# WhatAShot/Electrocardio-Panorama

Hardware: AMD Instinct MI355X
Metric: ECG-samples/sec (train step) (higher is better)
Workload: dtype f32 (conv products: fp32 operands split into fp16 hi+lo = 22-23 bits, block-scaled, 3 fp16 matrix products each, fp32 accumulate; fp32-class, not IEEE fp32)

## Files before the change

electrocardio_panorama_amd/_env.py:

```python
import os

PRODUCT = {
    "NEF_H2": "1 (default): K = 1 / 3 / 7 convolutions on the split-fp16 kernels; 0: the fp32 Winograd / direct kernels (strict fp32, "
              "required for data whose dynamic range exceeds ops.H2_HEADROOM per step)",
    "NEF_H2_TAIL": "warn (default): split-fp16 call sites whose operand is heavy-tailed (ops.H2_TAIL_FRAC) are counted and reported; "
                   "fp32: such WEIGHT-GRADIENT sites run on the fp32 kernels for their lifetime (per site, per rank)",
    "NEF_H2_ALLOW_CLAMP": "1: Solver warns instead of raising when a split-fp16 launch clamped outside a protected train step",
    "NEF_WINOGRAD": "fp32 path: 4 (default) F(4,.) forms where allowed, 2 / 1: F(2,.) only, 0: direct kernels only",
    "NEF_SIDE_STREAM": "auto (default) / 1 / 0: weight gradients on a second HIP stream",
    "NEF_SOLVER_GRAPH": "0: Solver never replays the captured step",
    "NEF_GRAPH_SPLIT": "0: data-parallel graphed step as ONE graph + one exposed all-reduce (default: two graphs, early bucket between them)",
    "NEF_EARLY_REDUCE": "0: eager data-parallel step reduces one bucket at the optimiser step (default: early bucket under the encoder's backward)",
    "NEF_BENCH_DUMP": "bench.py: file for the per-launch event times of the breakdown steps",
    "NEF_TIE_LOG": "tests: file for the tie ratios of the decision-replaying tests",
    "NEF_TEST_HOOKS": "1: honour the test hooks (TEST_HOOKS)",
}
TEST_HOOKS = {"NEF_SHARE_GPU", "NEF_DIST_BACKEND", "NEF_DIST_FORCE"}


def get(name, default=None):
    if name not in PRODUCT:
        raise KeyError(f"{name}: not a switch of this package (electrocardio_panorama_amd/_env.py)")
    return os.environ.get(name, default)
```

electrocardio_panorama_amd/_lib.py:

```python
import ctypes as C
import os

import torch

_HERE = os.path.dirname(os.path.abspath(__file__))
LIB_PATH = os.path.join(_HERE, "csrc", "libnefnet_hip.so")

NEF_OK = 0
_ERR = {-1: "NEF_E_SHAPE", -2: "NEF_E_NULL", -3: "NEF_E_WORKSPACE", -4: "NEF_E_UNSUPPORTED"}

p = C.c_void_p
i32 = C.c_int
i64 = C.c_int64
f32 = C.c_float
sz = C.c_size_t


class ConvArgs(C.Structure):
    _fields_ = [
        ("x", p), ("wp", p), ("y", p), ("bias", p), ("in_scale", p), ("res", p), ("gate", p), ("mask", p),
        ("x_bs", i64), ("x_gs", i64), ("y_bs", i64), ("y_gs", i64), ("sc_bs", i64), ("sc_gs", i64),
        ("res_bs", i64), ("res_gs", i64), ("gate_bs", i64), ("gate_gs", i64),
        ("B", i32), ("T", i32), ("G", i32), ("Cin_g", i32), ("Cout_g", i32), ("K", i32),
        ("relu", i32), ("gate_scale", f32), ("drop_scale", f32), ("drop_p", f32), ("rng_seed", C.c_uint64),
# ... 80 lines not shown


class LocateCandsArgs(C.Structure):
    _fields_ = [("best_theta", p), ("best_index", p), ("cands", p), ("s1", f32), ("s2", f32), ("ph1", f32), ("ph2", f32),
                ("B", i32), ("R", i32), ("radius", i32), ("reserved0", i32)]


class AugmentArgs(C.Structure):
    _fields_ = [("x", p), ("rois", p), ("y", p), ("seed_dev", p), ("seed", C.c_uint64),
                ("wander_amp", C.c_double), ("wander_lo", C.c_double), ("wander_hi", C.c_double), ("hum_amp", C.c_double),
                ("hum_hz", C.c_double), ("sample_rate", C.c_double), ("noise_std", f32), ("lead_drop", f32),
                ("B", i32), ("V", i32), ("L", i32), ("R", i32), ("crop", i32), ("reserved0", i32)]


class WarpArgs(C.Structure):
    _fields_ = [("data", p), ("target", p), ("rest", p), ("rois", p), ("data_out", p), ("target_out", p), ("rest_out", p),
                ("rois_out", p), ("seed", C.c_uint64), ("index0", i64), ("amp", C.c_double * 6),
                ("jitter", i32), ("B", i32), ("V", i32), ("R", i32), ("L", i32), ("reserved0", i32)]


class BeatBatchArgs(C.Structure):
    _fields_ = [("signal", p), ("plan", p), ("data", p), ("target_view", p), ("rest_view", p), ("signal_elems", i64),
                ("B", i32), ("V", i32), ("R", i32), ("dtype", i32)]


class BeatRangeArgs(C.Structure):
    _fields_ = [("signal", p), ("plan", p), ("range", p), ("signal_elems", i64), ("B", i32), ("V", i32), ("R", i32), ("dtype", i32)]


class BeatStitchArgs(C.Structure):
    _fields_ = [("views", p), ("range", p), ("table", p), ("out", p), ("view_bs", i64), ("view_as", i64), ("out_elems", i64),
                ("Bt", i32), ("A", i32), ("fill", i32), ("reserved0", i32)]


class RecordingStatsArgs(C.Structure):
    _fields_ = [("out", p), ("signal", p), ("beat_table", p), ("rec_table", p), ("out_offsets", p), ("score_leads", p), ("stats", p),
                ("out_elems", i64), ("signal_elems", i64), ("Bt", i32), ("N", i32), ("A", i32), ("fill", i32), ("dtype", i32),
                ("reserved0", i32)]


class PackDesc(C.Structure):
    _fields_ = [("w", p), ("wp", p), ("G", i32), ("Cog", i32), ("Cig", i32), ("K", i32), ("transpose_flip", i32),
                ("wino", i32), ("src_mode", i32), ("src_Cr", i32)]


SIGNATURES = {
    "nef_abi_version": (i32, []),
    "nef_debug_spin_us": (i32, [f32, i32, p]),
    "nef_stem_fwd": (i32, [p, p, p, i32, i32, i32, p]),
    "nef_stem_bwd_ws_bytes": (sz, [i32]),
    "nef_stem_bwd_weight": (i32, [p, p, p, p, p, sz, i32, i32, i32, p]),
    "nef_pack_weights": (i32, [C.POINTER(PackDesc), i32, p]),
    "nef_pack_bytes": (sz, [C.POINTER(PackDesc)]),
    "nef_conv_fwd": (i32, [C.POINTER(ConvArgs), p]),
    "nef_conv_args_bytes": (sz, []),
    "nef_conv_bwd_weight_ws_bytes": (sz, [C.POINTER(BwwArgs)]),
    "nef_conv_bwd_weight": (i32, [C.POINTER(BwwArgs), p]),
    "nef_bww_args_bytes": (sz, []),
    "nef_h2_tail_census_ws_bytes": (sz, [i32, i32, i32]),
    "nef_h2_tail_census": (i32, [p, i64, i64, i32, i32, i32, i32, p, i64, i64, p, p, i32, i32, p, f32, f32, p, sz, p, p, p, p]),
    "nef_bwd_weight_clamp_ends": (i32, [p, p, i64, i64, p, i32, i32, i32, i32, i32, p]),
    "nef_chan_sum_ws_bytes": (sz, [i32]),
    "nef_chan_sum": (i32, [p, p, p, sz, i32, i32, i32, p]),
    "nef_convt2_fwd": (i32, [p, p, p, p, i32, i32, i32, i32, i32, p]),
    "nef_convt2_bwd_data": (i32, [p, p, p, i32, i32, i32, i32, i32, p]),
    "nef_group_transpose": (i32, [p, p, i32, i32, i32, p]),
    "nef_convt2_interleave": (i32, [p, p, p, i32, i32, i32, p]),
    "nef_convt2_deinterleave": (i32, [p, p, i32, i32, i32, p]),
    "nef_convt2_bwd_weight_ws_bytes": (sz, [i32, i32, i32]),
    "nef_convt2_bwd_weight": (i32, [p, p, p, p, p, sz, i32, i32, i32, i32, i32, p]),
    "nef_theta_mlp_fwd": (i32, [p, p, p, p, i32, i32, p]),
    "nef_theta_mlp_bwd": (i32, [p, p, p, p, i32, i32, p]),
    "nef_theta_encode": (i32, [p, p, i32, p]),
    "nef_chscale_fwd": (i32, [p, p, i64, p, i32, i32, i32, p]),
    "nef_chscale_bwd": (i32, [p, p, p, i64, p, p, i32, i32, i32, i32, p]),
    "nef_gate": (i32, [p, p, p, f32, i64, p]),
    "nef_add": (i32, [p, p, p, i64, p]),
    "nef_roi_align_fwd": (i32, [p, p, p, i32, i32, i32, i32, i32, p]),
    "nef_roi_align_bwd": (i32, [p, p, p, i32, i32, i32, i32, i32, p]),
    "nef_window_crop": (i32, [p, i64, i64, p, i32, i32, i32, i32, i32, i32, p]),
    "nef_window_scatter": (i32, [p, p, i64, i64, i32, i32, i32, i32, i32, i32, p]),
    "nef_roi_unpool_fwd": (i32, [p, p, p, p, i32, i32, i32, p]),
    "nef_roi_unpool_bwd": (i32, [p, p, p, i32, i32, i32, p]),
    "nef_roi_segment_table": (i32, [p, p, p, i32, p]),
    "nef_lead_mean": (i32, [p, p, p, i32, i32, i32, p]),
    "nef_mix_fwd": (i32, [p, p, p, p, p, i32, i32, i32, i32, i32, p, p]),
    "nef_mix_bwd": (i32, [p, p, p, p, p, p, p, p, i32, i32, i32, i32, i32, p, i32, i32, i32, p]),
    "nef_mix_fwd_shared": (i32, [p, p, p, p, p, i32, i32, i32, i32, i32, p, p]),
    "nef_lead_mean_mix_shared": (i32, [p, p, p, p, p, i32, i32, i32, i32, i32, p, p]),
    "nef_lead_mean_mix_unpool": (i32, [p, p, p, p, p, p, p, i32, i32, i32, i32, i32, p, p]),
    "nef_mix_bwd_unpool": (i32, [p, p, p, p, p, p, p, p, p, i32, i32, i32, i32, i32, p, i32, p]),
    "nef_mix_bwd_unpool_rs": (i32, [p, p, p, p, p, p, p, p, p, p, p, sz, p, i32, i32, i32, i32, i32, p, i32, p]),
    "nef_mix_bwd_unpool_rs_ws_bytes": (sz, [i32, i32]),
    "nef_pass_combine_fwd": (i32, [p, p, p, i32, i32, i32, p]),
    "nef_pass_combine_bwd": (i32, [p, p, i32, i32, i32, p]),
    "nef_pass_combine_stats_ws_bytes": (sz, [i32, i32]),
    "nef_pass_combine_fwd_stats": (i32, [p, p, p, p, p, p, p, p, p, p, p, p, sz, i32, i32, i32, f32, f32, p, p]),
    "nef_upsample2_fwd": (i32, [p, p, i64, i32, p]),
    "nef_upsample2_bwd": (i32, [p, p, i64, i32, p]),
    "nef_bn_ws_bytes": (sz, [i32, i32]),
    "nef_bn_train_stats": (i32, [p, p, p, p, p, p, p, p, p, p, sz, i32, i32, i32, i32, f32, f32, p, p]),
    "nef_conv_stats_slots": (i32, [i32, i32]),
    "nef_bn_stats_from_slots": (i32, [p, i32, p, p, p, p, p, p, p, p, p, sz, i32, i32, i32, i32, f32, f32, p, p]),
    "nef_bn_eval_affine": (i32, [p, p, p, p, p, p, i32, f32, p]),
    "nef_fold_bn": (i32, [p, p, p, p, p, p, i32, i32, p]),
    "nef_affine_relu_fwd": (i32, [p, p, p, p, i32, i32, i32, i32, p]),
    "nef_bn_bwd_ws_bytes": (sz, [C.POINTER(BnBwdArgs)]),
    "nef_bn_relu_bwd": (i32, [C.POINTER(BnBwdArgs), p]),
    "nef_bn_bwd_args_bytes": (sz, []),
    "nef_bn_relu_bwd_outconv_w": (i32, [C.POINTER(BnBwdArgs), p, p, p, sz, p]),
# ... 141 lines not shown
```

electrocardio_panorama_amd/csrc/conv_h2.hip:

```cpp
#include <hip/hip_runtime.h>
#include <stdint.h>
#include <stdlib.h>

#include "nefnet_hip.h"
#include "nef_common.h"


typedef float f32x16 __attribute__((ext_vector_type(16)));
typedef float f32x4 __attribute__((ext_vector_type(4)));
typedef float f32x2 __attribute__((ext_vector_type(2)));
typedef float f32x4_a4 __attribute__((ext_vector_type(4), aligned(4)));
typedef _Float16 h16x8 __attribute__((ext_vector_type(8)));
typedef _Float16 h16x2 __attribute__((ext_vector_type(2)));
typedef unsigned u32x4 __attribute__((ext_vector_type(4)));
typedef unsigned u32x2 __attribute__((ext_vector_type(2)));

namespace {

constexpr int KC = 16;
constexpr int NTO = 256;
constexpr int PRO_MAX_CIN = 512;

__device__ __forceinline__ void split2(float x0, float x1, unsigned& h, unsigned& l) {
    x0 = __builtin_amdgcn_fmed3f(x0, -65000.f, 65000.f);
// ... 38 lines not shown
    const float* const wr = d.w + (r * d.Cig + ci) * 3;
    const float w0 = wr[0], w1 = wr[1], w2 = wr[2];
    if (p == 0) return kk == 0 ? fmaf(0.75f, w0, 0.25f * w1) : (kk == 1 ? fmaf(0.25f, w0, 0.75f * (w1 + w2)) : 0.25f * w2);
    return kk == 0 ? 0.25f * w0 : (kk == 1 ? fmaf(0.25f, w2, 0.75f * (w0 + w1)) : fmaf(0.75f, w2, 0.25f * w1));
}
constexpr int H2_PACK_MAX = 48;
struct H2PackTable { H2PackDesc d[H2_PACK_MAX]; };

__global__ __launch_bounds__(256) void pack_h2_kernel(H2PackTable tab) {
    const H2PackDesc& d = tab.d[blockIdx.y];
    const int co_n = d.flip ? d.Cig : d.Cog;
    const int ci_n = d.flip ? d.Cog : d.Cig;
    const int K = d.K;
    const int lane = threadIdx.x & 63;
    const int rows = d.G * co_n;
    const int ncot = co_n / 32, nc16 = ci_n / 16;
    float* const dsc = reinterpret_cast<float*>(d.wp + (int64_t)d.G * K * co_n * ci_n * 2);
    for (int row = blockIdx.x * 4 + (threadIdx.x >> 6); row < rows; row += gridDim.x * 4) {
        const int g = row / co_n, co = row % co_n;
        float m = 0.f;
        for (int i = lane; i < ci_n * K; i += 64) {
            const int ci = i / K, kk = i % K;
            const float v = d.flip ? h2_pack_src(d, (int64_t)g * d.Cog + ci, co, K - 1 - kk) : h2_pack_src(d, (int64_t)g * d.Cog + co, ci, kk);
            m = fmaxf(m, fabsf(v));
        }
#pragma unroll
        for (int o = 32; o > 0; o >>= 1) m = fmaxf(m, __shfl_xor(m, o, 64));
        int e = 0;
        if (m > 0.f && m < 3e38f) {
            int ex;
            (void)frexpf(m, &ex);
            e = 14 - (ex - 1);
            e = e > 100 ? 100 : (e < -100 ? -100 : e);
        }
        const float sc = ldexpf(1.f, e);
        if (lane == 0) dsc[row] = ldexpf(1.f, -e);
        for (int i = lane; i < ci_n * K; i += 64) {
            const int ci = i / K, kk = i % K;
            const float v = sc * (d.flip ? h2_pack_src(d, (int64_t)g * d.Cog + ci, co, K - 1 - kk) : h2_pack_src(d, (int64_t)g * d.Cog + co, ci, kk));
            const _Float16 h = (_Float16)v;
            const _Float16 l = (_Float16)(v - (float)h);
            const int64_t frag = ((((int64_t)g * nc16 + ci / 16) * K + kk) * ncot + co / 32) * 2;
            const int fl = (co & 31) + 32 * ((ci & 15) >> 3);
            d.wp[(frag * 64 + fl) * 8 + (ci & 7)] = h;
            d.wp[((frag + 1) * 64 + fl) * 8 + (ci & 7)] = l;
        }
    }
}

#define NEF_H2_TRACK1(V) amax_ = fmaxf(amax_, fabsf(V));
#define NEF_H2_TRACK2(V, W) amax_ = fmaxf(amax_, fmaxf(fabsf(V), fabsf(W)));
constexpr int H2_OCC1 = 3;
template <int K, int PRO, int TM, bool PACK = false>
__global__ __launch_bounds__(256, (TM == 1 && (PRO & 2) == 0) ? H2_OCC1 : 2) void conv_h2_kernel(nef_conv_args a_, int tps_, int n_tiles_, int m_tiles_) {
    constexpr int MT = 64 * TM;
    constexpr bool UP = (PRO & 2) != 0, AFF = (PRO & 1) != 0;
    constexpr bool PH = (PRO & 4) != 0;
    static_assert(!PH || (!UP && K == 3), "phase-stacked input: K = 3, no upsampling prologue");
    constexpr bool PF = (PRO & 8) != 0;
    static_assert(!PF || (!UP && !PH && K == 3 && TM == 2 && !PACK), "polyphase forward: K = 3, 128-row tile");
    constexpr int NS = UP ? 2 : 1;
    constexpr int PAD = (K - 1) / 2;
    constexpr int XROW = NTO + K - 1;
    constexpr int P4 = (XROW + 3) / 4 + 1;
    constexpr int PLANE = 4 * P4 * 32;
    constexpr int HALF = 4 * P4 * 16;
#define NEF_H2_WADDR(R, W) (((W) >> 1) * HALF + (((R) & 3) * P4 + ((R) >> 2)) * 16 + ((W) & 1) * 8)
#define NEF_H2_RPOS(S) ((((S) & 3) * P4 + ((S) >> 2)) * 16)
    constexpr int NIT = (XROW + 63) / 64;
    constexpr int NSF = K + 3;
    extern __shared__ __attribute__((aligned(16))) unsigned char smem_h2[];
    unsigned char* const Xl = smem_h2;
    float* const Pl = reinterpret_cast<float*>(smem_h2 + 4 * PLANE);
    float* const El = Pl + (AFF ? 2 * PRO_MAX_CIN : 0);
    float* const Al = El + 8 * MT;

    typedef const nef_conv_args __attribute__((address_space(4))) kargs_t;
    auto tile_pass = [&](kargs_t* const ap, const int bid, const int tid, const int tps, const int n_tiles, const int m_tiles,
                         const float xs_force, const bool last) __attribute__((always_inline)) -> float {
#define a (*ap)
    const int tile = bid % n_tiles;
    const int gm = bid / n_tiles;
    const int mt = gm % m_tiles;
    const int g = gm / m_tiles;
    int b0, t0;
    if constexpr (PACK) {
        b0 = tile * tps;
        t0 = 0;
    } else {
        const int full = (n_tiles / (8 * tps)) * (8 * tps);
        if (tile < full) {
            const int grp = tile / (8 * tps), r = tile % (8 * tps);
            b0 = grp * 8 + (r & 7);
            t0 = (r >> 3) * NTO;
        } else {
            b0 = tile / tps;
            t0 = (tile - b0 * tps) * NTO;
        }
    }
    const int m0 = mt * MT;
    const int T = a.T, Cig = a.Cin_g, Cog = a.Cout_g;
    const int lane = tid & 63, wave = tid >> 6;
    const int lo = lane & 31, hi = lane >> 5;
    const int wave_u = __builtin_amdgcn_readfirstlane(wave);
    const int wm = wave_u >> 1, wn = wave_u & 1;
    const int Tin = UP ? (T >> 1) : (PH ? 2 * T : T);

    const float* const xbase = a.x + (int64_t)b0 * a.x_bs + (int64_t)g * a.x_gs;
    const __amdgpu_buffer_rsrc_t xrs = nef_rsrc(xbase);
    const _Float16* const wph = reinterpret_cast<const _Float16*>(a.wp);
    const int ncot = Cog / 32, nc16 = Cig / 16;
    const __amdgpu_buffer_rsrc_t wrs = nef_rsrc(wph + ((int64_t)g * nc16 * K * ncot * 2 + (int64_t)(m0 / 32 + TM * wm) * 2) * 512);
    const unsigned a_tap = (unsigned)(ncot * 2 * 1024);

    const int64_t soff = (int64_t)b0 * a.sc_bs + (int64_t)g * a.sc_gs;
    float xs_ = xs_force;
    if (!last) {
        xs_ = a.x_scale != 0.f ? a.x_scale : 1.f;
        if (a.x_amax) {
            const float m_ = a.x_amax[0];
            if (m_ > 0.f && m_ < 3e38f) {
                int e_;
                (void)frexpf(m_, &e_);
                xs_ = ldexpf(1.f, 9 - e_ < 100 ? 9 - e_ : 100);
            }
        }
    }
    const int pro_row0 = AFF ? (b0 / a.pro_Bp) * a.G * Cig + g * Cig : 0;
    const unsigned avo = (unsigned)(lane * 16);
    unsigned xvo[NIT][NS];
    float lam[NIT];
    bool xok[NIT];
#pragma unroll
    for (int it = 0; it < NIT; ++it) {
        const int r = lane + 64 * it;
        const int t = t0 + r - PAD;
        xok[it] = (r < XROW) && (t >= 0) && (t < T);
        lam[it] = 0.f;
        if constexpr (PACK) {
            const int v = r - PAD, vb = v >= 0 ? v / (T + 4) : 0, tl = v - vb * (T + 4);
            xok[it] = (r < XROW) && v >= 0 && tl < T && vb < tps && b0 + vb < a.B;
            xvo[it][0] = xok[it] ? (unsigned)((vb * (int)a.x_bs + tl) * 4) : NEF_OOB;
        } else if constexpr (UP) {
            float src = 0.5f * ((float)t + 0.5f) - 0.5f;
            if (src < 0.f) src = 0.f;
            int i0 = (int)src;
            if (i0 > Tin - 1) i0 = Tin - 1;
            const int i1 = i0 + (i0 < Tin - 1 ? 1 : 0);
            lam[it] = src - (float)i0;
            xvo[it][0] = xok[it] ? (unsigned)(i0 * 4) : NEF_OOB;
            xvo[it][NS - 1] = xok[it] ? (unsigned)(i1 * 4) : NEF_OOB;
        } else if constexpr (PF) {
            xok[it] = (r < XROW) && (t >= -1) && (t <= T);
            const int tc = t < 0 ? 0 : (t > T - 1 ? T - 1 : t);
            xvo[it][0] = xok[it] ? (unsigned)(tc * 4) : NEF_OOB;
        } else {
            xvo[it][0] = xok[it] ? (unsigned)(t * (PH ? 8 : 4)) : NEF_OOB;
        }
    }
    unsigned uvo[2][2], mvo[2];
    bool uok[2][2], mok[2];
    float ulam[2];
    if constexpr (UP) {
        static_assert(!UP || (K == 3 && NTO == 256), "interval staging: K = 3, 256-column tiles");
#pragma unroll
// ... 116 lines not shown
                v *= sa_[rr];                                                                                       \
                NEF_H2_TRACK1(v)                                                                                    \
                v_[rr] = v;                                                                                         \
            }                                                                                                       \
            const int r = lane + 64 * it;                                                                           \
            unsigned h0_, l0_, h1_, l1_;                                                                            \
            split2n(v_[0], v_[1], h0_, l0_);                                                                        \
            split2n(v_[2], v_[3], h1_, l1_);                                                                        \
            const u32x2 hv = {h0_, h1_}, lv = {l0_, l1_};                                                           \
            if (r < XROW) {                                                                                         \
                unsigned char* p_ = (BUFP) + NEF_H2_WADDR(r, wave);                                                 \
                *reinterpret_cast<u32x2*>(p_) = hv;                                                                 \
                *reinterpret_cast<u32x2*>(p_ + PLANE) = lv;                                                         \
            }                                                                                                       \
        }                                                                                                           \
    }
    h16x8 fa[2][2 * TM];
#define NEF_H2A_ISSUE(CH, KK, SET)                                                                                   \
    {                                                                                                               \
        const unsigned so_ = (unsigned)(((CH) * K + (KK)) * a_tap);                                                 \
        _Pragma("unroll") for (int q = 0; q < 2 * TM; ++q)                                                          \
            fa[SET][q] = __builtin_bit_cast(h16x8, nef_buf_f32x4(wrs, avo, so_ + (unsigned)(q * 1024)));            \
    }

    NEF_H2X_ISSUE(0, xrs)
    NEF_H2A_ISSUE(0, 0, 0)
    if (tid < MT) {
        const int ch_ = g * Cog + m0 + (int)tid;
        const float* const dsc = reinterpret_cast<const float*>(wph + (int64_t)a.G * K * Cog * Cig * 2);
        if constexpr (PF) El[tid] = a.bias ? a.bias[g * (Cog >> 1) + (m0 >> 1) + ((int)tid >> 6) * 32 + ((int)tid & 31)] : 0.f;
        else
        El[tid] = a.bias ? a.bias[ch_] : 0.f;
        El[5 * MT + tid] = dsc[ch_] / xs_;
        El[6 * MT + tid] = (a.res_scale && b0 < a.B) ? a.res_scale[(int64_t)b0 * a.rs_bs + (int64_t)g * a.rs_gs + m0 + (int)tid] : 1.f;
        El[7 * MT + tid] = (a.gate_rowscale && b0 < a.B) ? a.gate_rowscale[(int64_t)b0 * a.gr_bs + (int64_t)g * a.gr_gs + m0 + (int)tid] : 1.f;
        if (a.bnb_slots) {
            const int pr_ = (b0 / a.bnb_Bp) * a.G * Cog + ch_;
            El[MT + tid] = a.bnb_mean[pr_];
            El[2 * MT + tid] = a.bnb_invstd[pr_];
            El[3 * MT + tid] = a.bnb_a[pr_];
            El[4 * MT + tid] = a.bnb_b[pr_];
        }
    }
    if constexpr (AFF) {
        for (int i = tid; i < Cig; i += 256) {
            Pl[i] = a.pro_a[pro_row0 + i];
            Pl[Cig + i] = a.pro_b[pro_row0 + i];
        }
        __syncthreads();
    }
    NEF_H2X_STORE(0, Xl)
    __syncthreads();

    const int nst = Cig / KC;
    const unsigned fb_lane = (unsigned)(hi * HALF + (wn * 32 + lo) * 16);
    for (int st = 0; st < nst; ++st) {
        const unsigned char* const xb = Xl + (st & 1) * (2 * PLANE) + fb_lane;
        const bool more = st + 1 < nst;
        const __amdgpu_buffer_rsrc_t xrs_n = nef_rsrc_n(xbase, more ? 0x7FFFFFFCu : 0u);
        h16x8 fb[5][2];
#define NEF_H2B_LOAD(S)                                                                                              \
    {                                                                                                               \
        const unsigned char* p_ = xb + NEF_H2_RPOS(S);                                                              \
        fb[(S) % 5][0] = *reinterpret_cast<const h16x8*>(p_);                                                       \
        fb[(S) % 5][1] = *reinterpret_cast<const h16x8*>(p_ + PLANE);                                               \
    }
        NEF_H2B_LOAD(0)
        NEF_H2B_LOAD(1)
        NEF_H2B_LOAD(2)
        NEF_H2B_LOAD(3)
#pragma unroll
        for (int kk = 0; kk < K; ++kk) {
            if (kk + 1 < K) NEF_H2A_ISSUE(st, kk + 1, (kk + 1) & 1)
            else NEF_H2A_ISSUE(more ? st + 1 : st, 0, (kk + 1) & 1)
            if (kk == 0) {
                __builtin_amdgcn_sched_barrier(0);
                NEF_H2X_ISSUE((st + 1) * KC, xrs_n)
            }
            if (kk + 4 < NSF) NEF_H2B_LOAD(kk + 4)
            __builtin_amdgcn_s_setprio(1);
            const int s_ = kk & 1;
#pragma unroll
            for (int j = 0; j < 4; ++j)
#pragma unroll
                for (int i = 0; i < TM; ++i)
                    acc[i][j] = __builtin_amdgcn_mfma_f32_32x32x16_f16(fa[s_][2 * i], fb[(kk + j) % 5][0], acc[i][j], 0, 0, 0);
#pragma unroll
            for (int j = 0; j < 4; ++j)
#pragma unroll
                for (int i = 0; i < TM; ++i)
                    acc[i][j] = __builtin_amdgcn_mfma_f32_32x32x16_f16(fa[s_][2 * i], fb[(kk + j) % 5][1], acc[i][j], 0, 0, 0);
#pragma unroll
            for (int j = 0; j < 4; ++j)
#pragma unroll
                for (int i = 0; i < TM; ++i)
                    acc[i][j] = __builtin_amdgcn_mfma_f32_32x32x16_f16(fa[s_][2 * i + 1], fb[(kk + j) % 5][0], acc[i][j], 0, 0, 0);
        }
#undef NEF_H2B_LOAD
        if constexpr ((K & 1) != 0) {
#pragma unroll
            for (int q = 0; q < 2 * TM; ++q) fa[0][q] = fa[1][q];
        }
        if (more) NEF_H2X_STORE((st + 1) * KC, Xl + ((st + 1) & 1) * (2 * PLANE))
        else {
#pragma unroll
            for (int o = 32; o > 0; o >>= 1) amax_ = fmaxf(amax_, __shfl_xor(amax_, o, 64));
            amax_ *= 1.f / xs_;
            if (lane == 0) Al[wave_u] = amax_;
        }
        __syncthreads();
    }
    {
        const float wg_ = fmaxf(fmaxf(Al[0], Al[1]), fmaxf(Al[2], Al[3]));
        if (!last && !(wg_ * xs_ < 65000.f) && wg_ < 3e38f) {
            __syncthreads();
            return wg_;
        }
    }
#undef NEF_H2X_ISSUE
#undef NEF_H2X_STORE
#undef NEF_H2A_ISSUE
#undef NEF_H2_WADDR
#undef NEF_H2_RPOS

    if (a.x_clamped && lane == 0 && !(amax_ * xs_ < 65000.f)) atomicAdd(a.x_clamped, 1);
    if (a.x_amax_next) {
        if (lane == 0 && amax_ < 3e38f) {
            unsigned* const p_ = reinterpret_cast<unsigned*>(a.x_amax_next);
            const unsigned b_ = __builtin_bit_cast(unsigned, amax_);
            if (b_ > __atomic_load_n(p_, __ATOMIC_RELAXED)) atomicMax(p_, b_);
        }
    }
    if constexpr (PF) {
        const int t = t0 + wn * 128 + 4 * lo;
        const bool inb = b0 < a.B;
        const bool live0 = inb && t < T, live1 = inb && t + 2 < T;
        const int Cr = Cog >> 1;
        const int cw = (m0 >> 1) + wm * 32;
        const int erow = wm * 64 + 4 * hi;
        const __amdgpu_buffer_rsrc_t yrs = nef_rsrc(a.y + (int64_t)b0 * a.y_bs + (int64_t)g * a.y_gs + (int64_t)cw * (2 * T));
        const unsigned yv0 = live0 ? (unsigned)((4 * hi * 2 * T + 2 * t) * 4) : NEF_OOB;
        const unsigned yv1 = live1 ? (unsigned)((4 * hi * 2 * T + 2 * t + 4) * 4) : NEF_OOB;
        float* const slot_out = a.stats;
        float sv[32];
#pragma unroll
        for (int h = 0; h < 2; ++h) {
#pragma unroll
            for (int q = 0; q < 8; ++q) {
                const int row = ((q + 8 * h) & 3) + 8 * ((q + 8 * h) >> 2);
                const float ds0 = El[5 * MT + erow + row], ds1 = El[5 * MT + erow + 32 + row], bv = El[erow + row];
                float y0[4], y1[4];
#pragma unroll
                for (int e = 0; e < 4; ++e) {
                    y0[e] = fmaf(acc[0][e][q + 8 * h], ds0, bv);
                    y1[e] = fmaf(acc[TM - 1][e][q + 8 * h], ds1, bv);
                }
                const f32x4 o0 = {y0[0], y1[0], y0[1], y1[1]}, o1 = {y0[2], y1[2], y0[3], y1[3]};
                nef_buf_store_f32x4(o0, yrs, yv0, (unsigned)(row * 2 * T * 4));
                nef_buf_store_f32x4(o1, yrs, yv1, (unsigned)(row * 2 * T * 4));
                if (slot_out) {
                    const float s0 = live0 ? (y0[0] + y1[0]) + (y0[1] + y1[1]) : 0.f, s1 = live1 ? (y0[2] + y1[2]) + (y0[3] + y1[3]) : 0.f;
                    const float q0 = live0 ? fmaf(y0[0], y0[0], y1[0] * y1[0]) + fmaf(y0[1], y0[1], y1[1] * y1[1]) : 0.f;
                    const float q1 = live1 ? fmaf(y0[2], y0[2], y1[2] * y1[2]) + fmaf(y0[3], y0[3], y1[3] * y1[3]) : 0.f;
                    sv[2 * (q + 8 * h)] = s0 + s1;
                    sv[2 * (q + 8 * h) + 1] = q0 + q1;
                }
// ... 192 lines not shown
            } else if (a.bnb_slots) {
                const float* xp = a.bnb_x + ((int64_t)b0 * ctot + (int64_t)g * Cog + cobase) * T;
#pragma unroll
                for (int q = 0; q < 8; ++q) {
                    const int row = NEF_ROW(q);
                    const int er = erow0 + row;
                    const float af = El[3 * MT + er], bf = El[4 * MT + er];
                    const float mf = El[MT + er], is = El[2 * MT + er];
                    const f32x2 x01 = *reinterpret_cast<const f32x2*>(xp + (int64_t)row * T + ts[0]);
                    const f32x2 x23 = *reinterpret_cast<const f32x2*>(xp + (int64_t)row * T + ts[1]);
                    const float g0 = (live[0] && fmaf(x01[0], af, bf) > 0.f) ? y[q][0] : 0.f;
                    const float g1 = (live[0] && fmaf(x01[1], af, bf) > 0.f) ? y[q][1] : 0.f;
                    const float g2 = (live[1] && fmaf(x23[0], af, bf) > 0.f) ? y[q][2] : 0.f;
                    const float g3 = (live[1] && fmaf(x23[1], af, bf) > 0.f) ? y[q][3] : 0.f;
                    sv[2 * (q + 8 * h)] = (g0 + g1) + (g2 + g3);
                    sv[2 * (q + 8 * h) + 1] = fmaf(g0, (x01[0] - mf) * is, g1 * ((x01[1] - mf) * is)) +
                                              fmaf(g2, (x23[0] - mf) * is, g3 * ((x23[1] - mf) * is));
                }
            } else if (a.stats && a.stats_mode == 0) {
#pragma unroll
                for (int q = 0; q < 8; ++q) {
                    const float y0 = live[0] ? y[q][0] : 0.f, y1 = live[0] ? y[q][1] : 0.f;
                    const float y2 = live[1] ? y[q][2] : 0.f, y3 = live[1] ? y[q][3] : 0.f;
                    sv[2 * (q + 8 * h)] = (y0 + y1) + (y2 + y3);
                    sv[2 * (q + 8 * h) + 1] = fmaf(y0, y0, y1 * y1) + fmaf(y2, y2, y3 * y3);
                }
            }
#undef NEF_ROW
        }
        if (slot_out) {
#pragma unroll
            for (int step = 0; step < 5; ++step) {
                const int off = 16 >> step;
                const bool up = (lo & off) != 0;
#pragma unroll
                for (int k = 0; k < off; ++k) {
                    const float send = up ? sv[k] : sv[k + off];
                    const float keep = up ? sv[k + off] : sv[k];
                    sv[k] = keep + __shfl_xor(send, off, 64);
                }
            }
            const int r = lo >> 1;
            const int ch = g * Cog + cobase + (r & 3) + 8 * (r >> 2);
            const int64_t nslot = (int64_t)tps * 2;
            const int64_t slot = (int64_t)b0 * nslot + (int64_t)(t0 / NTO) * 2 + wn;
            if (inb) slot_out[((int64_t)ch * a.B * nslot + slot) * 2 + (lo & 1)] = sv[0];
        }
    }
    return -1.f;
#undef a
    };
    kargs_t* ap_ = (kargs_t*)__builtin_amdgcn_kernarg_segment_ptr();
    (void)a_;
    const float over_ = tile_pass(ap_, (int)blockIdx.x, (int)threadIdx.x, tps_, n_tiles_, m_tiles_, 0.f, false);
    if (over_ > 0.f) {
        int e_;
        (void)frexpf(over_, &e_);
        int bid_ = (int)blockIdx.x, tid_ = (int)threadIdx.x, tps2_ = tps_, nt2_ = n_tiles_, mt2_ = m_tiles_;
        asm volatile("" : "+s"(ap_), "+s"(bid_), "+s"(tps2_), "+s"(nt2_), "+s"(mt2_));
        asm volatile("" : "+v"(tid_));
        (void)tile_pass(ap_, bid_, tid_, tps2_, nt2_, mt2_, ldexpf(1.f, 9 - e_ < 100 ? 9 - e_ : 100), true);
    }
}

template <int K, int PRO, int TM, bool PACK = false>
int launch_h2(const nef_conv_args& a, hipStream_t st) {
    constexpr int MT = 64 * TM;
    constexpr int XROW = NTO + K - 1;
    constexpr int P4 = (XROW + 3) / 4 + 1;
    constexpr int PLANE = 4 * P4 * 32;
    constexpr size_t lds = (size_t)4 * PLANE + (((PRO & 1) ? 2 * PRO_MAX_CIN : 0) + 8 * MT + 4) * sizeof(float);
    static unsigned long long lds_set = 0;
    if (int e = nef_ensure_dyn_lds(reinterpret_cast<const void*>(&conv_h2_kernel<K, PRO, TM, PACK>), lds, &lds_set)) return e;
    const int tps = PACK ? (NTO + 4) / (a.T + 4) : (a.T + NTO - 1) / NTO;
    const int n_tiles = PACK ? (a.B + tps - 1) / tps : a.B * tps;
    const int m_tiles = a.Cout_g / MT;
    const int64_t blocks = (int64_t)a.G * m_tiles * n_tiles;
    if (blocks <= 0 || blocks > 0x7fffffff) return NEF_E_SHAPE;
    hipLaunchKernelGGL((conv_h2_kernel<K, PRO, TM, PACK>), dim3((unsigned)blocks), dim3(256), lds, st, a, tps, n_tiles, m_tiles);
    return nef_launch_status();
}

}

static bool h2_pack_shape(const nef_conv_args* a) {
    if (!(a->T >= 8 && a->T <= 64 && a->T % 4 == 0 && (a->K == 1 || a->K == 3))) return false;
    const int64_t spt = (NTO + 4) / (a->T + 4);
    const int64_t lim = 0x7fffffff / 4;
    return a->pro_mode == 0 && !a->in_scale && !a->res_scale && !a->gate_rowscale && !a->stats && !a->bnb_slots && spt * a->x_bs < lim && spt * a->y_bs < lim &&
           (!a->res || spt * a->res_bs < lim) && (!a->gate || spt * a->gate_bs < lim);
}

__attribute__((visibility("hidden"))) bool nef_h2_ok(const nef_conv_args* a) {
    return (a->K == 1 || a->K == 3 || a->K == 7) && a->Cout_g % 64 == 0 && a->Cin_g % KC == 0 && a->T % 2 == 0 &&
           (a->T >= NTO / 2 || h2_pack_shape(a)) &&
           ((a->pro_mode >= 0 && a->pro_mode <= 4) || a->pro_mode == 8 || a->pro_mode == 9) && (a->K == 3 || a->pro_mode == 0) &&
           !(a->pro_mode && a->in_scale) &&
           (!a->res_scale || (a->res && !(a->pro_mode & 8))) &&
           ((!a->gate_rowscale && a->stats_mode == 0) || (a->gate && !(a->pro_mode & 8) && (a->stats_mode == 0 || (a->stats_mode == 1 && a->stats && !a->bnb_slots)))) &&
           (!(a->pro_mode & 8) || (a->Cout_g % 128 == 0 && a->T >= NTO / 2 && !a->res && !a->gate && !a->mask && !a->relu && a->drop_p <= 0.f &&
                                   !a->bnb_slots && (int64_t)a->Cout_g * a->T * 4 < 0x7fffffff)) &&
           (a->pro_mode != 4 || (a->T >= NTO / 2 && (int64_t)a->Cin_g * a->T * 4 < 0x7fffffff)) &&
           (!(a->pro_mode & 1) || a->Cin_g <= PRO_MAX_CIN);
}

__attribute__((visibility("hidden"))) int nef_h2_launch(const nef_conv_args* a, hipStream_t st) {
    if (!nef_h2_ok(a)) return NEF_E_SHAPE;
    if ((a->pro_mode & 1) && !(a->pro_a && a->pro_b && a->pro_Bp > 0)) return NEF_E_NULL;
    const bool wide = a->Cout_g % 128 == 0;
    if (a->T < NTO / 2)
        return a->K == 1 ? launch_h2<1, 0, 1, true>(*a, st) : launch_h2<3, 0, 1, true>(*a, st);
    if (a->K == 7) return wide ? launch_h2<7, 0, 2>(*a, st) : launch_h2<7, 0, 1>(*a, st);
    if (a->K == 1) return wide ? launch_h2<1, 0, 2>(*a, st) : launch_h2<1, 0, 1>(*a, st);
    switch (a->pro_mode) {
        case 0: return wide ? launch_h2<3, 0, 2>(*a, st) : launch_h2<3, 0, 1>(*a, st);
        case 1: return wide ? launch_h2<3, 1, 2>(*a, st) : launch_h2<3, 1, 1>(*a, st);
        case 2: return launch_h2<3, 2, 1>(*a, st);
        case 4: return wide ? launch_h2<3, 4, 2>(*a, st) : launch_h2<3, 4, 1>(*a, st);
        case 8: return launch_h2<3, 8, 2>(*a, st);
        case 9: return launch_h2<3, 9, 2>(*a, st);
        default: return launch_h2<3, 3, 1>(*a, st);
    }
}

__attribute__((visibility("hidden"))) int nef_h2_pack_status(const nef_pack_desc* dp) {
    const nef_pack_desc& d = *dp;
    const int co_n = d.transpose_flip ? d.Cig : d.Cog, ci_n = d.transpose_flip ? d.Cog : d.Cig;
    if (d.G <= 0 || co_n % 32 != 0 || ci_n % 16 != 0 || (d.K != 1 && d.K != 3 && d.K != 7)) return NEF_E_SHAPE;
    if (d.src_mode != 0 && !(d.src_mode == 1 && d.K == 3 && d.Cog % 2 == 0 && d.src_Cr >= 0 &&
                             (d.src_Cr == 0 || (d.src_Cr % 64 == 0 && d.Cog == 2 * d.src_Cr)))) return NEF_E_SHAPE;
    return NEF_OK;
}

__attribute__((visibility("hidden"))) int nef_h2_pack(const nef_pack_desc* descs, int n, hipStream_t st) {
    for (int i0 = 0; i0 < n; i0 += H2_PACK_MAX) {
        H2PackTable tab;
        const int m = n - i0 < H2_PACK_MAX ? n - i0 : H2_PACK_MAX;
        int rows_max = 1;
        for (int i = 0; i < m; ++i) {
            const nef_pack_desc& d = descs[i0 + i];
            if (!d.w || !d.wp) return NEF_E_NULL;
            if (int e = nef_h2_pack_status(&d)) return e;
            const int co_n = d.transpose_flip ? d.Cig : d.Cog;
            tab.d[i] = H2PackDesc{d.w, reinterpret_cast<_Float16*>(d.wp), d.G, d.Cog, d.Cig, d.K, d.transpose_flip, d.src_mode, d.src_Cr};
            if (d.G * co_n > rows_max) rows_max = d.G * co_n;
        }
        hipLaunchKernelGGL(pack_h2_kernel, dim3((unsigned)((rows_max + 3) / 4), (unsigned)m), dim3(256), 0, st, tab);
    }
    return nef_launch_status();
}
```

electrocardio_panorama_amd/csrc/conv_h2w.hip:

```cpp
#include <hip/hip_runtime.h>
#include <stdint.h>
#include <stdlib.h>

#include <type_traits>

#include "nefnet_hip.h"
#include "nef_common.h"


typedef float f32x16 __attribute__((ext_vector_type(16)));
typedef float f32x2 __attribute__((ext_vector_type(2)));
typedef _Float16 h16x8 __attribute__((ext_vector_type(8)));
typedef _Float16 h16x2 __attribute__((ext_vector_type(2)));
typedef unsigned u32x4 __attribute__((ext_vector_type(4)));
typedef unsigned u32x2 __attribute__((ext_vector_type(2)));

namespace {

constexpr int TT = 64;
constexpr int GP = TT * 2 + 8;
constexpr int XW = TT + 8;
constexpr int XP = XW * 2 + 8;
constexpr int X_PLANE = 64 * XP;
constexpr int gy_plane(int MCO) { return 64 * MCO * GP; }
constexpr int buf_bytes(int MCO) { return 2 * gy_plane(MCO) + 2 * X_PLANE; }

struct H2WArgs {
    const float* x;
    const float* gy;
    const float* in_scale;
    const float* pro_a;
    const float* pro_b;
    float* ws;
    const float* x_amax;
    const float* gy_amax;
    float* x_amax_next;
    float* gy_amax_next;
    int* clamped;
    int64_t x_bs, x_gs, gy_bs, gy_gs, sc_bs, sc_gs;
    int64_t x_end, gy_end;
    int B, T, G, Cig, Cog, pro_Bp, S, tps, n_tiles, m_tiles, c_tiles, teams;
    float x_scale, gy_scale;
    int xclamp;
};


__device__ __forceinline__ void split_pair_s(float x0, float x1, float s, unsigned& h, unsigned& l) {
    asm("v_fma_mixlo_f16 %0, %1, %2, 0 op_sel:[0,0,0] op_sel_hi:[0,0,0]" : "=v"(h) : "v"(x0), "v"(s));
    asm("v_fma_mixhi_f16 %0, %1, %2, 0 op_sel:[0,0,0] op_sel_hi:[0,0,0]" : "+v"(h) : "v"(x1), "v"(s));
    asm("v_fma_mixlo_f16 %0, %1, %2, -%3 op_sel:[0,0,0] op_sel_hi:[0,0,1]" : "=v"(l) : "v"(x0), "v"(s), "v"(h));
    asm("v_fma_mixhi_f16 %0, %1, %2, -%3 op_sel:[0,0,1] op_sel_hi:[0,0,1]" : "+v"(l) : "v"(x1), "v"(s), "v"(h));
}
__device__ __forceinline__ void split_one_s(float x0, float s, unsigned& h, unsigned& l) {
    asm("v_fma_mixlo_f16 %0, %1, %2, 0 op_sel:[0,0,0] op_sel_hi:[0,0,0]" : "=v"(h) : "v"(x0), "v"(s));
    asm("v_fma_mixlo_f16 %0, %1, %2, -%3 op_sel:[0,0,0] op_sel_hi:[0,0,1]" : "=v"(l) : "v"(x0), "v"(s), "v"(h));
}

__device__ __forceinline__ float scale_for(float m) {
    int e;
    (void)frexpf(m, &e);
    return ldexpf(1.f, 9 - e);
}

__device__ __forceinline__ float scale_from(const float* amax, float fallback) {
    float s = fallback != 0.f ? fallback : 1.f;
    if (amax) {
        const float m = amax[0];
        if (m > 0.f && m < 3e38f) {
            int e;
            (void)frexpf(m, &e);
            s = ldexpf(1.f, 9 - e);
        }
    }
    return s;
}

template <int K, int K0, int K1, int MCO, int KA>
__device__ __forceinline__ void h2w_chunk(const unsigned char* ga, const unsigned char* xa, int c, f32x16 (&acc)[MCO][KA]) {
    constexpr int PAD = (K - 1) / 2;
    constexpr int GY_PLANE = gy_plane(MCO);
    h16x8 fah[MCO], fal[MCO];
#pragma unroll
    for (int i = 0; i < MCO; ++i) {
        unsigned ah[4], al[4];
#pragma unroll
        for (int j = 0; j < 2; ++j) {
            const u32x2 vh = *reinterpret_cast<const u32x2*>(ga + i * 32 * GP + c * 32 + 8 * j);
            const u32x2 vl = *reinterpret_cast<const u32x2*>(ga + i * 32 * GP + GY_PLANE + c * 32 + 8 * j);
            ah[2 * j] = vh[0], ah[2 * j + 1] = vh[1];
            al[2 * j] = vl[0], al[2 * j + 1] = vl[1];
        }
        fah[i] = __builtin_bit_cast(h16x8, u32x4{ah[0], ah[1], ah[2], ah[3]});
        fal[i] = __builtin_bit_cast(h16x8, u32x4{al[0], al[1], al[2], al[3]});
    }
    unsigned wh[8], wl[8];
#pragma unroll
    for (int j = 0; j < 4; ++j) {
// ... 303 lines not shown
        if (e0 & 1) {
            fbh[k] = __builtin_bit_cast(h16x8, u32x4{wo_h[d], wo_h[d + 1], wo_h[d + 2], wo_h[d + 3]});
            fbl[k] = __builtin_bit_cast(h16x8, u32x4{wo_l[d], wo_l[d + 1], wo_l[d + 2], wo_l[d + 3]});
        } else {
            fbh[k] = __builtin_bit_cast(h16x8, u32x4{wn_h[d], wn_h[d + 1], wn_h[d + 2], wn_h[d + 3]});
            fbl[k] = __builtin_bit_cast(h16x8, u32x4{wn_l[d], wn_l[d + 1], wn_l[d + 2], wn_l[d + 3]});
        }
    }
#pragma unroll
    for (int i = 0; i < WR; ++i)
#pragma unroll
        for (int k = 0; k < K; ++k) acc[i][k] = __builtin_amdgcn_mfma_f32_32x32x16_f16(fah[i], fbh[k], acc[i][k], 0, 0, 0);
#pragma unroll
    for (int i = 0; i < WR; ++i)
#pragma unroll
        for (int k = 0; k < K; ++k) acc[i][k] = __builtin_amdgcn_mfma_f32_32x32x16_f16(fal[i], fbh[k], acc[i][k], 0, 0, 0);
#pragma unroll
    for (int i = 0; i < WR; ++i)
#pragma unroll
        for (int k = 0; k < K; ++k) acc[i][k] = __builtin_amdgcn_mfma_f32_32x32x16_f16(fah[i], fbl[k], acc[i][k], 0, 0, 0);
}

template <int K, int PRO, int WM, int WN, int WR, int TTv, int NP, int DEPTH>
__global__ __launch_bounds__(64 * (WM / WR * WN + NP), 1) void conv_h2w2_kernel(H2WArgs a) {
    constexpr bool UP = (PRO & 2) != 0, AFF = (PRO & 1) != 0;
    constexpr int NC = WM / WR * WN;
    constexpr int NT = 64 * NP, RG = 32 * WM, RX = 32 * WN;
    constexpr int GP = TTv * 2 + 16, XE = TTv + 8, XP = XE * 2;
    constexpr int G_PLANE = RG * GP, X_PLANE = RX * XP, BUF = 2 * G_PLANE + 4 * X_PLANE;
    constexpr int QG = TTv / 4, QX = XE / 4, NGQ = RG * QG / NT, NXQ = (RX * QX + NT - 1) / NT, NCH = TTv / 16;
    constexpr int GROWS = NT / QG;
    static_assert(RG * QG % NT == 0 && GP % 32 == 16 && XP % 32 == 16, "tile form");
    extern __shared__ __attribute__((aligned(16))) unsigned char smem_w[];

    const int members = a.m_tiles * a.c_tiles;
    const int xcd = blockIdx.x & 7, q_ = blockIdx.x >> 3;
    const int member = q_ % members;
    const int team = (q_ / members) * 8 + xcd;
    if (team >= a.teams) return;
    const int g = team / a.S, sp = team % a.S;
    const int mt = member / a.c_tiles, ct = member % a.c_tiles;
    const int T = a.T, Tin = UP ? (T >> 1) : T;
    const int lane = (int)threadIdx.x & 63;
    const int lo = lane & 31, hi = lane >> 5;
    const int wave_u = __builtin_amdgcn_readfirstlane((int)threadIdx.x >> 6);
    const int wm = (wave_u % NC) / WN * WR, wn = wave_u % WN;
    const bool producer = wave_u >= NC;
    const int tid = ((int)threadIdx.x - 64 * NC) & (NT - 1);

    const int64_t per = ((int64_t)a.n_tiles + a.S - 1) / a.S;
    const int n_lo = (int)(per * sp);
    int n_hi = (int)(per * (sp + 1));
    if (n_hi > a.n_tiles) n_hi = a.n_tiles;

    float* const Wl = reinterpret_cast<float*>(smem_w);
    float rx_ = 0.f, rg_ = 0.f;
    auto share_pass = [&](const float sx, const float sg, const bool last) __attribute__((always_inline)) -> bool {
    float amax_x = 0.f, amax_g = 0.f;

    f32x16 acc[WR][K];
#pragma unroll
    for (int i = 0; i < WR; ++i)
#pragma unroll
        for (int k = 0; k < K; ++k)
#pragma unroll
            for (int r = 0; r < 16; ++r) acc[i][k][r] = 0.f;

    const int g_row = tid / QG, g_qd = tid % QG;
    const unsigned g_voff = (unsigned)((g_row * T + 4 * g_qd) * 4);
    const unsigned g_lds = (unsigned)(g_row * GP + g_qd * 8);
    unsigned x_voff[NXQ], x_lds[NXQ], x_row[NXQ], x_qd[NXQ];
#pragma unroll
    for (int q = 0; q < NXQ; ++q) {
        const int p = tid + NT * q;
        const int row = p < RX * QX ? p / QX : 0, qd = p < RX * QX ? p % QX : 0;
        x_row[q] = (unsigned)row, x_qd[q] = (unsigned)qd;
        x_voff[q] = p < RX * QX ? (unsigned)((row * Tin + (UP ? 2 : 4) * qd) * 4) : NEF_OOB;
        x_lds[q] = (unsigned)(row * XP + qd * 8);
    }
    const bool has_sc = a.in_scale != nullptr;

    struct Stage {
        f32x4 gq[NGQ];
        f32x4 xq[NXQ];
        float x5[NXQ], ppa[NXQ], ppb[NXQ], psc[NXQ];
    };
    Stage st0, st1;

    auto is_edge = [&](int N) { const int t0_ = (N % a.tps) * TTv; return !(t0_ > 0 && t0_ + TTv + 6 <= T); };

    auto issue = [&](Stage& z, int N, auto edge_c, int part) __attribute__((always_inline)) {
        constexpr bool EDGE = decltype(edge_c)::value;
        const int b_ = N / a.tps, t0_ = (N % a.tps) * TTv;
        const bool on_ = N < n_hi;
        const int64_t goff = (int64_t)b_ * a.gy_bs + (int64_t)g * a.gy_gs + (int64_t)(mt * RG) * T + (EDGE ? 0 : t0_);
        const __amdgpu_buffer_rsrc_t grs = nef_rsrc_n(a.gy + goff, extent_from(a.gy_end, goff, on_));
#pragma unroll
        for (int q = 0; q < ((part & 1) ? NGQ : 0); ++q) {
            const unsigned so = (unsigned)(q * GROWS * T * 4);
            if constexpr (!EDGE) {
                z.gq[q] = nef_buf_f32x4(grs, g_voff, so);
            } else {
#pragma unroll
                for (int i = 0; i < 4; ++i) {
                    const int t = t0_ + 4 * g_qd + i;
                    z.gq[q][i] = nef_buf_f32(grs, t < T ? g_voff + (unsigned)((t0_ + i) * 4) : NEF_OOB, so);
                }
            }
        }
        const int64_t xrow0 = (int64_t)b_ * a.x_bs + (int64_t)g * a.x_gs + (int64_t)(ct * RX) * Tin;
        const int64_t xoff = xrow0 + (EDGE ? 0 : (UP ? (t0_ - 4) / 2 - 1 : t0_ - 4));
        const __amdgpu_buffer_rsrc_t xrs = nef_rsrc_n(a.x + xoff, extent_from(a.x_end, xoff, on_));
#pragma unroll
        for (int q = 0; q < ((part & 2) ? NXQ : 0); ++q) {
            if constexpr (!EDGE) {
                z.xq[q] = nef_buf_f32x4(xrs, x_voff[q], 0);
                if constexpr (!UP) z.x5[q] = nef_buf_f32(xrs, x_voff[q], 16);
            } else {
                const unsigned rowoff = x_voff[q] - (unsigned)((UP ? 2 : 4) * 4) * x_qd[q];
                const bool live = x_voff[q] != NEF_OOB;
                const int t = t0_ - 4 + 4 * (int)x_qd[q];
                if constexpr (UP) {
                    const int h_ = t >> 1;
#pragma unroll
                    for (int i = 0; i < 4; ++i) {
                        int c_ = h_ - 1 + i;
                        c_ = c_ < 0 ? 0 : (c_ > Tin - 1 ? Tin - 1 : c_);
                        z.xq[q][i] = nef_buf_f32(xrs, live && t + 4 >= 0 && t < T ? rowoff + (unsigned)(c_ * 4) : NEF_OOB, 0);
                    }
                } else {
#pragma unroll
                    for (int i = 0; i < 5; ++i) {
                        int ti = t + i;
                        if (a.xclamp) ti = ti == -1 ? 0 : (ti == T ? T - 1 : ti);
                        const float v = nef_buf_f32(xrs, live && ti >= 0 && ti < T ? rowoff + (unsigned)(ti * 4) : NEF_OOB, 0);
                        if (i < 4) z.xq[q][i] = v; else z.x5[q] = v;
                    }
                }
            }
            const int bq = on_ ? b_ : 0;
            if constexpr (AFF) {
                const int pr = (bq / a.pro_Bp) * a.G * a.Cig + g * a.Cig + ct * RX;
                z.ppa[q] = a.pro_a[pr + (int)x_row[q]], z.ppb[q] = a.pro_b[pr + (int)x_row[q]];
            }
            if (has_sc) z.psc[q] = a.in_scale[(int64_t)bq * a.sc_bs + (int64_t)g * a.sc_gs + ct * RX + (int)x_row[q]];
        }
    };

    auto store = [&](Stage& z, int N, unsigned char* bufp, auto edge_c, int part) __attribute__((always_inline)) {
        constexpr bool EDGE = decltype(edge_c)::value;
        const int t0_ = (N % a.tps) * TTv;
#pragma unroll
        for (int q = 0; q < ((part & 1) ? NGQ : 0); ++q) {
            const f32x4 v = z.gq[q];
            amax_g = fmaxf(amax_g, fmaxf(fabsf(v[0]), fabsf(v[1])));
            amax_g = fmaxf(amax_g, fmaxf(fabsf(v[2]), fabsf(v[3])));
            unsigned h0, l0, h1, l1;
            split_pair_s(v[0], v[1], sg, h0, l0);
            split_pair_s(v[2], v[3], sg, h1, l1);
            unsigned char* p_ = bufp + g_lds + q * GROWS * GP;
            *reinterpret_cast<u32x2*>(p_) = u32x2{h0, h1};
            *reinterpret_cast<u32x2*>(p_ + G_PLANE) = u32x2{l0, l1};
        }
#pragma unroll
        for (int q = 0; q < ((part & 2) ? NXQ : 0); ++q) {
            if (tid + NT * q < RX * QX) {
                float v[5];
                if constexpr (UP) {
                    float s0 = z.xq[q][0], s1 = z.xq[q][1], s2 = z.xq[q][2], s3 = z.xq[q][3];
                    if constexpr (AFF) {
                        s0 = fmaxf(fmaf(s0, z.ppa[q], z.ppb[q]), 0.f), s1 = fmaxf(fmaf(s1, z.ppa[q], z.ppb[q]), 0.f);
                        s2 = fmaxf(fmaf(s2, z.ppa[q], z.ppb[q]), 0.f), s3 = fmaxf(fmaf(s3, z.ppa[q], z.ppb[q]), 0.f);
                    }
                    v[0] = (1.f - 0.75f) * s0 + 0.75f * s1;
                    v[1] = (1.f - 0.25f) * s1 + 0.25f * s2;
                    v[2] = (1.f - 0.75f) * s1 + 0.75f * s2;
                    v[3] = (1.f - 0.25f) * s2 + 0.25f * s3;
                    v[4] = (1.f - 0.75f) * s2 + 0.75f * s3;
                    if constexpr (EDGE) {
                        if (t0_ - 4 + 4 * (int)x_qd[q] == 0) v[0] = s1;
                        if (t0_ + 4 * (int)x_qd[q] == 0) v[4] = s3;
                    }
                } else {
                    v[0] = z.xq[q][0], v[1] = z.xq[q][1], v[2] = z.xq[q][2], v[3] = z.xq[q][3], v[4] = z.x5[q];
                    if constexpr (AFF) {
#pragma unroll
                        for (int i = 0; i < 5; ++i) v[i] = fmaxf(fmaf(v[i], z.ppa[q], z.ppb[q]), 0.f);
                    }
                }
                if (has_sc) {
#pragma unroll
                    for (int i = 0; i < 5; ++i) v[i] *= z.psc[q];
                }
                if constexpr (EDGE) {
                    const int t = t0_ - 4 + 4 * (int)x_qd[q];
                    const int lo_ = a.xclamp ? -1 : 0, hi_ = a.xclamp ? T + 1 : T;
#pragma unroll
                    for (int i = 0; i < 5; ++i)
                        if (t + i < lo_ || t + i >= hi_) v[i] = 0.f;
                }
                amax_x = fmaxf(amax_x, fmaxf(fabsf(v[0]), fabsf(v[1])));
                amax_x = fmaxf(amax_x, fmaxf(fabsf(v[2]), fabsf(v[3])));
                unsigned h0, l0, h1, l1, h2, l2;
                split_pair_s(v[0], v[1], sx, h0, l0);
// ... 100 lines not shown
        for (int k = 0; k < K; ++k)
#pragma unroll
            for (int r = 0; r < 16; ++r) wsp[((int64_t)k * a.Cog + co0 + (r & 3) + 8 * (r >> 2)) * a.Cig + ci] = acc[i][k][r] * ds;
    }
    return true;
    };
    const float sx0 = scale_from(a.x_amax, a.x_scale), sg0 = scale_from(a.gy_amax, a.gy_scale);
    if (!share_pass(sx0, sg0, false))
        (void)share_pass(rx_ * sx0 < 65000.f ? sx0 : scale_for(rx_), rg_ * sg0 < 65000.f ? sg0 : scale_for(rg_), true);
}

template <int K, int PRO, int WM, int WN, int WR, int TTv, int NP, int DEPTH>
int launch_h2w2(const H2WArgs& a, hipStream_t st) {
    constexpr size_t lds = 2 * (2 * (32 * WM) * (TTv * 2 + 16) + 4 * (32 * WN) * ((TTv + 8) * 2));
    static unsigned long long lds_set = 0;
    if (int e = nef_ensure_dyn_lds(reinterpret_cast<const void*>(&conv_h2w2_kernel<K, PRO, WM, WN, WR, TTv, NP, DEPTH>), lds, &lds_set)) return e;
    const int members = a.m_tiles * a.c_tiles;
    const int teams8 = (a.teams + 7) / 8 * 8;
    const int64_t blocks = (int64_t)teams8 * members;
    if (blocks <= 0 || blocks > 0x7fffffff) return NEF_E_SHAPE;
    hipLaunchKernelGGL((conv_h2w2_kernel<K, PRO, WM, WN, WR, TTv, NP, DEPTH>), dim3((unsigned)blocks), dim3(64 * (WM / WR * WN + NP)), lds, st, a);
    return nef_launch_status();
}

int h2w2_form(int Cog, int pro_mode) {
    if (Cog % 128 == 0) return 1;
    return ((H2W2_64_MODES >> pro_mode) & 1) ? 2 : 0;
}

}

extern "C" {

__attribute__((visibility("hidden"))) bool nef_h2w_ok(int B, int T, int Cig, int Cog, int K, int pro_mode) {
    return (K == 1 || K == 3 || K == 7) && B > 0 && T >= TT && T % 2 == 0 && Cig % 64 == 0 && Cog % 64 == 0 && pro_mode >= 0 &&
           (pro_mode <= 3 || (pro_mode <= 5 && Cog % 128 == 0)) && (K == 3 || pro_mode == 0);
}

__attribute__((visibility("hidden"))) int nef_h2w_splits(int B, int T, int G, int Cig, int Cog, int K, int pro_mode, int* partials) {
    const int v2 = h2w2_form(Cog, pro_mode & 3);
    const H2WForm f = h2w_form(Cog, K);
    const int tps = (T + TT - 1) / TT;
    const int64_t n_tiles = (int64_t)B * tps;
    const int units = v2 ? G * (Cog / (v2 == 1 ? 128 : 64)) * (Cig / 64) : G * (Cog / (64 * f.mco)) * (Cig / 64);
    const int resident = v2 ? 1 : (f.split ? 1 : 2);
    const int slots = resident * nef_cu_count();
    int S = slots / units;
    if (S > n_tiles) S = (int)n_tiles;
    if (S < 1) S = 1;
    if (partials) *partials = S * (!v2 && f.split == 2 ? 2 : 1);
    return S;
}

__attribute__((visibility("hidden"))) int nef_h2w_launch(const nef_bww_args& b, int S, hipStream_t st) {
    const int B = b.B, T = b.T, G = b.G, Cig = b.Cin_g, Cog = b.Cout_g, K = b.K;
    int pro_mode = b.pro_mode;
    if (!nef_h2w_ok(B, T, Cig, Cog, K, pro_mode)) return NEF_E_SHAPE;
    if ((b.x_amax_next == nullptr) != (b.gy_amax_next == nullptr)) return NEF_E_NULL;
    const H2WForm f = h2w_form(Cog, K);
    H2WArgs a;
    a.x = b.x, a.gy = b.gy, a.in_scale = b.in_scale, a.pro_a = b.pro_a, a.pro_b = b.pro_b, a.ws = (float*)b.ws;
    a.x_amax = b.x_amax, a.gy_amax = b.gy_amax, a.x_amax_next = b.x_amax_next, a.gy_amax_next = b.gy_amax_next, a.clamped = b.clamped;
    a.x_bs = b.x_bs, a.x_gs = b.x_gs, a.gy_bs = b.gy_bs, a.gy_gs = b.gy_gs, a.sc_bs = b.sc_bs, a.sc_gs = b.sc_gs;
    a.B = B, a.T = T, a.G = G, a.Cig = Cig, a.Cog = Cog, a.pro_Bp = b.pro_Bp, a.S = S;
    a.tps = (T + TT - 1) / TT;
    a.n_tiles = B * a.tps;
    a.m_tiles = Cog / (64 * f.mco), a.c_tiles = Cig / 64;
    a.teams = G * S;
    a.x_scale = b.x_scale, a.gy_scale = b.gy_scale;
    a.xclamp = (pro_mode >> 2) & 1;
    pro_mode &= 3;
    const int Tin = (pro_mode & 2) ? T / 2 : T;
    a.x_end = ((int64_t)(B - 1) * b.x_bs + (int64_t)(G - 1) * b.x_gs + (int64_t)Cig * Tin) * 4;
    a.gy_end = ((int64_t)(B - 1) * b.gy_bs + (int64_t)(G - 1) * b.gy_gs + (int64_t)Cog * T) * 4;
    if (a.xclamp && !h2w2_form(Cog, pro_mode)) return NEF_E_UNSUPPORTED;
    if (const int v2 = h2w2_form(Cog, pro_mode)) {
        a.m_tiles = Cog / (v2 == 1 ? 128 : 64), a.c_tiles = Cig / 64;
#define NEF_H2W2(KK, PP)                                                                                             \
    (v2 == 1 ? launch_h2w2<KK, PP, 4, 2, (KK == 7 ? 1 : 2), 64, (KK == 7 ? 4 : 8), (KK == 7 ? 1 : 2)>(a, st)               \
             : launch_h2w2<KK, PP, 2, 2, 1, 64, 8, (KK == 7 ? 1 : 2)>(a, st))
        if (K == 7) return NEF_H2W2(7, 0);
        if (K == 1) return NEF_H2W2(1, 0);
        switch (pro_mode) {
            case 0: return NEF_H2W2(3, 0);
            case 1: return NEF_H2W2(3, 1);
            case 2: return NEF_H2W2(3, 2);
            default: return NEF_H2W2(3, 3);
        }
#undef NEF_H2W2
    }
    if (K == 7) return launch_h2w<7, 0, 1, 0>(a, st);
    if (K == 1) return launch_h2w<1, 0, 1, 0>(a, st);
    return pro_mode == 0 ? launch_h2w<3, 0, 1, 0>(a, st) : launch_h2w<3, 1, 1, 0>(a, st);
}

}
```

electrocardio_panorama_amd/csrc/conv_mfma.hip:

```cpp
#include "nef_common.h"
#include <stdlib.h>

typedef float f32x16 __attribute__((ext_vector_type(16)));
typedef float f32x4 __attribute__((ext_vector_type(4)));
typedef float f32x2 __attribute__((ext_vector_type(2)));

#ifndef NEF_MFMA_PART
#define NEF_MFMA_PART 0
#endif
#define NEF_PART(n) (NEF_MFMA_PART == 0 || NEF_MFMA_PART == (n))

namespace {

constexpr int NT = 128;
constexpr int WT = 64;

template <int K> struct StageK;
template <> struct StageK<7> { static constexpr int KC = 16; };
template <int K, int TM> struct FwdStage {
    static constexpr int KC = ((K == 7 || K == 3) && TM == 2) ? 8 : StageK<K>::KC;
};
template <> struct StageK<3> { static constexpr int KC = 16; };
template <> struct StageK<1> { static constexpr int KC = 64; };

// ... 1882 lines not shown
        else pack_plain_elem(d.w, d.wp, d.G, d.Cog, d.Cig, d.K, d.transpose_flip, i);
    }
}

__global__ void chan_sum_partial(const float* __restrict__ x, double* __restrict__ part, int B, int C, int T,
                                 int nsplit) {
    __shared__ double sm[4];
    const int c = blockIdx.x % C;
    const int sp = blockIdx.x / C;
    double s = 0.0;
    const int nb = sp < B ? (B - sp + nsplit - 1) / nsplit : 0;
    if (T >= 512 && (T & 1) == 0) {
        const int T2 = T >> 1;
        int bi = 0;
        for (; bi + 4 <= nb; bi += 4) {
            const float2* r0 = reinterpret_cast<const float2*>(x + ((int64_t)(sp + bi * nsplit) * C + c) * T);
            const int64_t rs = (int64_t)nsplit * C * T2;
            for (int t = threadIdx.x; t < T2; t += blockDim.x) {
                const float2 a0 = r0[t], a1 = r0[rs + t], a2 = r0[2 * rs + t], a3 = r0[3 * rs + t];
                s += ((double)a0.x + (double)a0.y) + ((double)a1.x + (double)a1.y) +
                     (((double)a2.x + (double)a2.y) + ((double)a3.x + (double)a3.y));
            }
        }
        for (; bi < nb; ++bi) {
            const float2* r0 = reinterpret_cast<const float2*>(x + ((int64_t)(sp + bi * nsplit) * C + c) * T);
            for (int t = threadIdx.x; t < T2; t += blockDim.x) {
                const float2 a0 = r0[t];
                s += (double)a0.x + (double)a0.y;
            }
        }
    } else {
        for (int i = threadIdx.x; i < nb * T; i += blockDim.x) {
            const int bi = i / T, t = i - bi * T;
            s += (double)x[((int64_t)(sp + bi * nsplit) * C + c) * T + t];
        }
    }
    s = nef_block_sum_d(s, sm);
    if (threadIdx.x == 0) part[(int64_t)sp * C + c] = s;
}

__global__ void chan_sum_final(const double* __restrict__ part, float* __restrict__ out, int C, int nsplit) {
    const int c = blockIdx.x * blockDim.x + threadIdx.x;
    if (c >= C) return;
    double s = 0.0;
    for (int sp = 0; sp < nsplit; ++sp) s += part[(int64_t)sp * C + c];
    out[c] = (float)s;
}

constexpr int CHAN_SUM_SPLIT = 16;

}

__attribute__((visibility("hidden"))) bool nef_h2_ok(const nef_conv_args* a);
__attribute__((visibility("hidden"))) int nef_h2_launch(const nef_conv_args* a, hipStream_t st);
__attribute__((visibility("hidden"))) int nef_h2_pack(const nef_pack_desc* descs, int n, hipStream_t st);
__attribute__((visibility("hidden"))) int nef_h2_pack_status(const nef_pack_desc* d);

__attribute__((visibility("hidden"))) int nef_mfma_wino4_fwd(const nef_conv_args* a, hipStream_t st);
__attribute__((visibility("hidden"))) int nef_mfma_wino_fwd(const nef_conv_args* a, hipStream_t st);

#if NEF_PART(1)
extern "C" {

int nef_abi_version(void) { return 22; }

static int pack_desc_status(const nef_pack_desc& d) {
    NEF_REQUIRE(d.G > 0 && d.Cog > 0 && d.Cig > 0 && d.K > 0 && d.wino >= 0 && d.wino <= 3 &&
                    (!d.wino || d.K == 3 || d.K == 7 || (d.wino == 3 && d.K == 1)), NEF_E_SHAPE);
    NEF_REQUIRE(d.src_mode == 0 || d.wino == 3, NEF_E_UNSUPPORTED);
    return NEF_OK;
}

size_t nef_pack_bytes(const nef_pack_desc* d) {
    if (!d || pack_desc_status(*d) || (d->wino == 3 && nef_h2_pack_status(d))) return 0;
    static const int planes[3][2] = {{0, 0}, {4, 10}, {6, 13}};
    const size_t e = (size_t)d->G * d->Cog * d->Cig;
    if (d->wino == 3) return (e * d->K + (size_t)d->G * (d->transpose_flip ? d->Cig : d->Cog)) * sizeof(float);
    return e * (d->wino ? planes[d->wino][d->K == 7] : d->K) * sizeof(float);
}

int nef_pack_weights(const nef_pack_desc* descs, int n, nef_stream_t stream) {
    NEF_ENTER();
    NEF_REQUIRE(descs || n == 0, NEF_E_NULL);
    NEF_REQUIRE(n >= 0, NEF_E_SHAPE);
    nef_pack_desc h2[PACK_MULTI_MAX];
    int n_h2 = 0, n_f32 = 0;
    for (int i = 0; i < n; ++i) {
        const nef_pack_desc& d = descs[i];
        NEF_REQUIRE(d.w && d.wp, NEF_E_NULL);
        if (int e = pack_desc_status(d)) return e;
        if (d.wino == 3) {
            if (n_h2 == PACK_MULTI_MAX) {
                if (int e = nef_h2_pack(h2, n_h2, (hipStream_t)stream)) return e;
                n_h2 = 0;
            }
            h2[n_h2++] = d;
        } else {
            ++n_f32;
        }
    }
    if (n_h2) {
        if (int e = nef_h2_pack(h2, n_h2, (hipStream_t)stream)) return e;
    }
    for (int i0 = 0; i0 < n;) {
        PackTable t;
        int m = 0;
        int64_t biggest = 1;
        for (; i0 < n && m < PACK_MULTI_MAX; ++i0) {
            if (descs[i0].wino == 3) continue;
            t.d[m++] = descs[i0];
        }
        if (m == 0) break;
        for (int i = 0; i < m; ++i) {
            const int64_t e = (int64_t)t.d[i].G * t.d[i].Cog * t.d[i].Cig * (t.d[i].wino ? 1 : t.d[i].K);
            if (e > biggest) biggest = e;
        }
        int gx = (int)nef_cdiv(biggest, 256);
        if (n_f32 == 1) gx = nef_stream_grid(biggest, 256);
        else if (gx > 64) gx = 64;
        hipLaunchKernelGGL(pack_weights_multi_kernel, dim3((unsigned)gx, (unsigned)m), dim3(256), 0, (hipStream_t)stream, t);
    }
    return nef_launch_status();
}

size_t nef_conv_args_bytes(void) { return sizeof(nef_conv_args); }


int nef_conv_fwd(const nef_conv_args* a, nef_stream_t stream) {
    NEF_ENTER();
    NEF_REQUIRE(a && a->x && a->wp && a->y, NEF_E_NULL);
    NEF_REQUIRE(a->B > 0 && a->T > 0 && a->G > 0, NEF_E_SHAPE);
    const int K = a->K;
    NEF_REQUIRE(K == 1 || K == 3 || K == 7, NEF_E_SHAPE);
    NEF_REQUIRE(a->Cout_g % 64 == 0 && a->Cin_g > 0, NEF_E_SHAPE);
    hipStream_t st = (hipStream_t)stream;
    NEF_REQUIRE((!a->stats && !a->bnb_slots) || a->wino == 2 || a->wino == 3, NEF_E_UNSUPPORTED);
    NEF_REQUIRE(!(a->stats && a->bnb_slots), NEF_E_UNSUPPORTED);
    NEF_REQUIRE(!a->bnb_slots || (a->bnb_x && a->bnb_mean && a->bnb_invstd && a->bnb_a && a->bnb_b), NEF_E_NULL);
    NEF_REQUIRE(!a->bnb_slots || a->bnb_Bp > 0, NEF_E_SHAPE);
    NEF_REQUIRE(!a->bnb_slots || !a->bnb_up || a->T % 4 == 0, NEF_E_SHAPE);
    NEF_REQUIRE((!a->res_scale && !a->gate_rowscale && a->stats_mode == 0) || a->wino == 3, NEF_E_UNSUPPORTED);
    if (a->wino == 3) {
        NEF_REQUIRE(nef_h2_ok(a), NEF_E_SHAPE);
        return nef_h2_launch(a, st);
    }
    bool big = (a->Cout_g % 128 == 0);
    if (big) {
        const ColTiling ct0 = make_tiling(a->B, a->T, NT);
        if ((int64_t)a->G * (a->Cout_g / 128) * ct0.n_tiles < 384) big = false;
    }
    const int KC = K == 1 ? FwdStage<1, 1>::KC : (big ? FwdStage<3, 2>::KC : FwdStage<3, 1>::KC);
    static_assert(FwdStage<7, 2>::KC == FwdStage<3, 2>::KC && FwdStage<7, 1>::KC == FwdStage<3, 1>::KC, "stage sizes");
    NEF_REQUIRE(a->Cin_g % KC == 0, NEF_E_SHAPE);
    if (a->wino == 2) return nef_mfma_wino4_fwd(a, st);
    if (a->wino) return nef_mfma_wino_fwd(a, st);
    if (a->pro_mode != 0) {
        NEF_REQUIRE(K == 3 && a->pro_mode >= 1 && a->pro_mode <= 3 && !a->in_scale, NEF_E_UNSUPPORTED);
        NEF_REQUIRE(!(a->pro_mode & 1) || (a->pro_a && a->pro_b && a->pro_Bp > 0), NEF_E_NULL);
        NEF_REQUIRE(!(a->pro_mode & 2) || (a->T % 2 == 0), NEF_E_SHAPE);
        if (a->pro_mode & 1) {
            const ColTiling ct = make_tiling(a->B, a->T, NT);
            NEF_REQUIRE(ct.nseg == 1 || a->pro_Bp % ct.nseg == 0, NEF_E_SHAPE);
        }
        switch (a->pro_mode) {
            case 1: return big ? launch_conv_fwd<3, 2, 1>(*a, st) : launch_conv_fwd<3, 1, 1>(*a, st);
            case 2: return big ? launch_conv_fwd<3, 2, 2>(*a, st) : launch_conv_fwd<3, 1, 2>(*a, st);
            default: return big ? launch_conv_fwd<3, 2, 3>(*a, st) : launch_conv_fwd<3, 1, 3>(*a, st);
        }
    }
    switch (K) {
        case 7: return big ? launch_conv_fwd<7, 2>(*a, st) : launch_conv_fwd<7, 1>(*a, st);
        case 3: return big ? launch_conv_fwd<3, 2>(*a, st) : launch_conv_fwd<3, 1>(*a, st);
        default: return big ? launch_conv_fwd<1, 2>(*a, st) : launch_conv_fwd<1, 1>(*a, st);
    }
}

int nef_conv_stats_slots(int T, int Cout_g) {
    if (T <= 0 || T % 2 != 0 || Cout_g <= 0 || Cout_g % 64 != 0) return 0;
    const bool wide = (Cout_g % 128 == 0);
    if (T < (wide ? 128 : 256)) return 0;
    const int nto = wide ? 128 : 256;
    return ((T + nto - 1) / nto) * (nto / 128);
}

size_t nef_bww_args_bytes(void) { return sizeof(nef_bww_args); }

size_t nef_conv_bwd_weight_ws_bytes(const nef_bww_args* a) {
    if (!a) return 0;
    const int B = a->B, T = a->T, G = a->G, Cin_g = a->Cin_g, Cout_g = a->Cout_g, K = a->K;
    int partials = 0;
    if (a->form == 0 || a->form == 4) {
        BwdWeightPlan p;
        if (!plan_bwd_weight(B, T, G, Cin_g, Cout_g, K, &p)) return 0;
        partials = p.S;
    } else if (a->form == 3) {
        if (G <= 0 || !nef_h2w_ok(B, T, Cin_g, Cout_g, K, 0)) return 0;
        for (int pm = 0; pm < (K == 3 ? 4 : 1); ++pm) {
            int p_ = 0;
            (void)nef_h2w_splits(B, T, G, Cin_g, Cout_g, K, pm, &p_);
            if (p_ > partials) partials = p_;
        }
    }
    return (size_t)partials * G * K * Cout_g * Cin_g * sizeof(float);
}

static int bww_direct(const nef_bww_args& a, hipStream_t st, int* S_used) {
    const int K = a.K, pro_mode = a.pro_mode;
    NEF_REQUIRE(a.B > 0 && a.T > 0 && a.G > 0, NEF_E_SHAPE);
    NEF_REQUIRE(pro_mode == 0 || (K == 3 && pro_mode >= 1 && pro_mode <= 3 && !a.in_scale), NEF_E_UNSUPPORTED);
    NEF_REQUIRE(!(pro_mode & 2) || (a.T % 2 == 0), NEF_E_SHAPE);
    BwdWeightPlan p;
    NEF_REQUIRE(plan_bwd_weight(a.B, a.T, a.G, a.Cin_g, a.Cout_g, K, &p, pro_mode), NEF_E_SHAPE);
    NEF_REQUIRE(!(pro_mode & 1) || p.ct.nseg == 1 || a.pro_Bp % p.ct.nseg == 0, NEF_E_SHAPE);
    const size_t need = (size_t)p.S * a.G * K * a.Cout_g * a.Cin_g * sizeof(float);
    NEF_REQUIRE(a.ws_bytes >= need, NEF_E_WORKSPACE);
    int rc = NEF_E_UNSUPPORTED;
#define NEF_BW(KK, WCO, TCI) rc = launch_bwd_weight<KK, WCO, TCI>(p, a, st)
#define NEF_BWP(WCO, TCI)                                                                                              \
    {                                                                                                                 \
        if (pro_mode == 0) NEF_BW(3, WCO, TCI);                                                                       \
        else if (pro_mode == 1) rc = launch_bwd_weight<3, WCO, TCI, 1>(p, a, st);                                     \
        else if (pro_mode == 2) rc = launch_bwd_weight<3, WCO, TCI, 2>(p, a, st);                                     \
        else rc = launch_bwd_weight<3, WCO, TCI, 3>(p, a, st);                                                        \
    }
    if (K == 7) {
        if (p.wco == 4) NEF_BW(7, 4, 1); else NEF_BW(7, 2, 1);
    } else if (K == 3) {
        if (p.wco == 4) { if (p.tci == 2) NEF_BWP(4, 2) else NEF_BWP(4, 1) }
        else if (p.tci == 2) NEF_BW(3, 2, 2);
        else NEF_BWP(2, 1)
    } else {
        if (p.wco == 4) { if (p.tci == 2) NEF_BW(1, 4, 2); else NEF_BW(1, 4, 1); }
        else { if (p.tci == 2) NEF_BW(1, 2, 2); else NEF_BW(1, 2, 1); }
    }
#undef NEF_BWP
#undef NEF_BW
    *S_used = p.S;
    return rc;
}

static int bww_h2(const nef_bww_args& a, hipStream_t st, int* S_used) {
    NEF_REQUIRE(a.G > 0 && nef_h2w_ok(a.B, a.T, a.Cin_g, a.Cout_g, a.K, a.pro_mode), NEF_E_SHAPE);
    NEF_REQUIRE(!(a.pro_mode && a.in_scale), NEF_E_UNSUPPORTED);
    const int S = nef_h2w_splits(a.B, a.T, a.G, a.Cin_g, a.Cout_g, a.K, a.pro_mode, S_used);
    NEF_REQUIRE(a.ws_bytes >= (size_t)*S_used * a.G * a.K * a.Cout_g * a.Cin_g * sizeof(float), NEF_E_WORKSPACE);
    return nef_h2w_launch(a, S, st);
}

int nef_conv_bwd_weight(const nef_bww_args* args, nef_stream_t stream) {
    NEF_ENTER();
    NEF_REQUIRE(args && args->x && args->gy && args->gw && args->ws, NEF_E_NULL);
    nef_bww_args a = *args;
    if (!(a.pro_mode & 1) && a.pro_Bp <= 0) a.pro_Bp = 1;
    NEF_REQUIRE(!(a.pro_mode & 1) || (a.pro_a && a.pro_b && a.pro_Bp > 0), NEF_E_NULL);
    hipStream_t st = (hipStream_t)stream;
    int S = 0, rc;
    switch (a.form) {
        case 0: rc = bww_direct(a, st, &S); break;
        case 4: rc = nef_mfma_bww_wino4(a, st, &S); break;
        case 3: rc = bww_h2(a, st, &S); break;
        default: return NEF_E_UNSUPPORTED;
    }
    if (rc != NEF_OK) return rc;
    const int64_t n = (int64_t)a.G * a.K * a.Cout_g * a.Cin_g;
    hipLaunchKernelGGL(conv_bwd_weight_reduce, dim3(nef_stream_grid(n, 256)), dim3(256), 0, st, (const float*)a.ws, a.gw, a.G,
                       a.Cout_g, a.Cin_g, a.K, S);
    return nef_launch_status();
}

size_t nef_chan_sum_ws_bytes(int C) { return (size_t)CHAN_SUM_SPLIT * C * sizeof(double); }

int nef_chan_sum(const float* x, float* out, void* ws, size_t ws_bytes, int B, int C, int T, nef_stream_t stream) {
    NEF_ENTER();
    NEF_REQUIRE(x && out && ws, NEF_E_NULL);
    NEF_REQUIRE(B > 0 && C > 0 && T > 0, NEF_E_SHAPE);
    NEF_REQUIRE(ws_bytes >= nef_chan_sum_ws_bytes(C), NEF_E_WORKSPACE);
    hipStream_t st = (hipStream_t)stream;
    hipLaunchKernelGGL(chan_sum_partial, dim3(C * CHAN_SUM_SPLIT), dim3(256), 0, st, x, (double*)ws, B, C, T,
                       CHAN_SUM_SPLIT);
    hipLaunchKernelGGL(chan_sum_final, dim3((C + 255) / 256), dim3(256), 0, st, (const double*)ws, out, C,
                       CHAN_SUM_SPLIT);
    return nef_launch_status();
}

}
#endif

#if NEF_PART(2)
__attribute__((visibility("hidden"))) int nef_mfma_wino4_fwd(const nef_conv_args* a, hipStream_t st) {
    const int K = a->K;
        NEF_REQUIRE((K == 3 || K == 7) && a->T % 2 == 0 && a->Cin_g % WKC == 0, NEF_E_SHAPE);
        NEF_REQUIRE(a->pro_mode >= 0 && a->pro_mode <= 3 && !(a->pro_mode && a->in_scale), NEF_E_UNSUPPORTED);
        NEF_REQUIRE(K == 3 || a->pro_mode == 0, NEF_E_UNSUPPORTED);
        NEF_REQUIRE(!(a->pro_mode & 1) || (a->pro_a && a->pro_b && a->pro_Bp > 0), NEF_E_NULL);
        const bool wide = (a->Cout_g % 128 == 0);
        NEF_REQUIRE(a->T >= (wide ? 128 : 256), NEF_E_SHAPE);
        if (K == 7) return wide ? launch_conv_wino4<7, 4, 0>(*a, st) : launch_conv_wino4<7, 2, 0>(*a, st);
        switch (a->pro_mode) {
            case 0: return wide ? launch_conv_wino4<3, 4, 0>(*a, st) : launch_conv_wino4<3, 2, 0>(*a, st);
            case 1: return wide ? launch_conv_wino4<3, 4, 1>(*a, st) : launch_conv_wino4<3, 2, 1>(*a, st);
            case 2: return wide ? launch_conv_wino4<3, 4, 2>(*a, st) : launch_conv_wino4<3, 2, 2>(*a, st);
            default: return wide ? launch_conv_wino4<3, 4, 3>(*a, st) : launch_conv_wino4<3, 2, 3>(*a, st);
        }
}
#endif

#if NEF_PART(3)
__attribute__((visibility("hidden"))) int nef_mfma_wino_fwd(const nef_conv_args* a, hipStream_t st) {
    const int K = a->K;
        NEF_REQUIRE((K == 3 || K == 7) && a->T % 2 == 0 && a->Cin_g % WKC == 0, NEF_E_SHAPE);
        NEF_REQUIRE(a->pro_mode >= 0 && a->pro_mode <= 3 && !(a->pro_mode && a->in_scale), NEF_E_UNSUPPORTED);
        NEF_REQUIRE(K == 3 || a->pro_mode == 0, NEF_E_UNSUPPORTED);
        NEF_REQUIRE(!(a->pro_mode & 1) || (a->pro_a && a->pro_b && a->pro_Bp > 0), NEF_E_NULL);
        const bool wide = (a->Cout_g % 128 == 0);
        NEF_REQUIRE(a->T >= (wide ? 128 : 256), NEF_E_SHAPE);
        if (K == 7) return wide ? launch_conv_wino<7, 2, 0>(*a, st) : launch_conv_wino<7, 1, 0>(*a, st);
        switch (a->pro_mode) {
            case 0: return wide ? launch_conv_wino<3, 2, 0>(*a, st) : launch_conv_wino<3, 1, 0>(*a, st);
            case 1: return wide ? launch_conv_wino<3, 2, 1>(*a, st) : launch_conv_wino<3, 1, 1>(*a, st);
            case 2: return wide ? launch_conv_wino<3, 2, 2>(*a, st) : launch_conv_wino<3, 1, 2>(*a, st);
// ... 47 lines not shown
```

electrocardio_panorama_amd/csrc/nef_common.h:

```cpp
#pragma once
#include <hip/hip_runtime.h>
#include <stdint.h>

#include "nefnet_hip.h"

#define NEF_WAVE 64

#define NEF_REQUIRE(cond, code) \
    do {                        \
        if (!(cond)) return (code); \
    } while (0)

#define NEF_ENTER() (void)hipGetLastError()

static inline int nef_launch_status() {
    hipError_t e = hipGetLastError();
    return e == hipSuccess ? NEF_OK : (int)e;
}

static inline int64_t nef_cdiv(int64_t a, int64_t b) { return (a + b - 1) / b; }

static inline int nef_cu_count() {
    static int cached[64] = {0};
    int dev = 0;
// ... 45 lines not shown
    return sm[0] + sm[1] + sm[2] + sm[3];
}

__device__ __forceinline__ int nef_row_end(const int64_t* __restrict__ rois, int i, int L) {
    if (!rois) return L;
    const int64_t e = rois[(int64_t)i * 14 + 12];
    return e < 0 ? 0 : (e > L ? L : (int)e);
}

__device__ __forceinline__ uint64_t nef_rng_mix(uint64_t seed, uint64_t pair) {
    uint64_t z = pair + seed * 0x9E3779B97F4A7C15ull + 0x632BE59BD9B4E019ull;
    z = (z ^ (z >> 30)) * 0xBF58476D1CE4E5B9ull;
    z = (z ^ (z >> 27)) * 0x94D049BB133111EBull;
    return z ^ (z >> 31);
}
__device__ __forceinline__ float nef_rng_uniform(uint64_t seed, uint64_t idx) {
    const uint64_t z = nef_rng_mix(seed, idx >> 1);
    return (float)((idx & 1) ? ((z >> 16) & 0xFFFFFFull) : (z >> 40)) * (1.0f / 16777216.0f);
}
__device__ __forceinline__ void nef_rng_uniform2(uint64_t seed, uint64_t even_idx, float& u0, float& u1) {
    const uint64_t z = nef_rng_mix(seed, even_idx >> 1);
    u0 = (float)(z >> 40) * (1.0f / 16777216.0f);
    u1 = (float)((z >> 16) & 0xFFFFFFull) * (1.0f / 16777216.0f);
}

typedef unsigned nef_u32x4 __attribute__((ext_vector_type(4)));
typedef float nef_f32x4 __attribute__((ext_vector_type(4)));
#define NEF_OOB 0x80000000u

__device__ __forceinline__ __amdgpu_buffer_rsrc_t nef_rsrc(const void* p) {
    return __builtin_amdgcn_make_buffer_rsrc(const_cast<void*>(p), 0, 0x7FFFFFFC, 0x00020000);
}
__device__ __forceinline__ __amdgpu_buffer_rsrc_t nef_rsrc_n(const void* p, unsigned bytes) {
    return __builtin_amdgcn_make_buffer_rsrc(const_cast<void*>(p), 0, (int)bytes, 0x00020000);
}
__device__ __forceinline__ float nef_buf_f32(__amdgpu_buffer_rsrc_t r, unsigned voff, unsigned soff) {
    return __builtin_bit_cast(float, __builtin_amdgcn_raw_buffer_load_b32(r, (int)voff, (int)soff, 0));
}
typedef float nef_f32x2 __attribute__((ext_vector_type(2)));
__device__ __forceinline__ nef_f32x2 nef_buf_f32x2(__amdgpu_buffer_rsrc_t r, unsigned voff, unsigned soff) {
    return __builtin_bit_cast(nef_f32x2, __builtin_amdgcn_raw_buffer_load_b64(r, (int)voff, (int)soff, 0));
}
__device__ __forceinline__ void nef_buf_store_f32x4(nef_f32x4 v, __amdgpu_buffer_rsrc_t r, unsigned voff, unsigned soff) {
    __builtin_amdgcn_raw_buffer_store_b128(__builtin_bit_cast(nef_u32x4, v), r, (int)voff, (int)soff, 0);
}
__device__ __forceinline__ nef_f32x4 nef_buf_f32x4(__amdgpu_buffer_rsrc_t r, unsigned voff, unsigned soff) {
    return __builtin_bit_cast(nef_f32x4, __builtin_amdgcn_raw_buffer_load_b128(r, (int)voff, (int)soff, 0));
}

#define NEF_HIDDEN __attribute__((visibility("hidden")))
extern "C" {
NEF_HIDDEN bool nef_h2w_ok(int B, int T, int Cig, int Cog, int K, int pro_mode);
NEF_HIDDEN int nef_h2w_splits(int B, int T, int G, int Cig, int Cog, int K, int pro_mode, int* partials);
NEF_HIDDEN int nef_h2w_launch(const nef_bww_args& a, int S, hipStream_t st);
NEF_HIDDEN bool nef_bww_glds_ok(const nef_bww_args& a);
NEF_HIDDEN int nef_bww_glds_launch(const nef_bww_args& a, int half, int S_max, int fixed_S, int* S_used, hipStream_t st);
}
NEF_HIDDEN int nef_mfma_bww_wino4(const nef_bww_args& a, hipStream_t st, int* S_used);
```

electrocardio_panorama_amd/csrc/stem.hip:

```cpp
#include "nef_common.h"

namespace {

constexpr int KW = 15;
constexpr int TP = 64;
constexpr int CPL = 128;

__device__ __forceinline__ void load_window(__amdgpu_buffer_rsrc_t xrow, int L, int tp, float (&xw)[19]) {
    const int base = 4 * tp - 9;
#pragma unroll
    for (int i = 0; i < 19; ++i) {
        const int p = base + i;
        xw[i] = nef_buf_f32(xrow, (p >= 0 && p < L) ? (unsigned)(p * 4) : NEF_OOB, 0);
    }
}

constexpr int FWD_TP = TP - 1;

__global__ __launch_bounds__(256) void stem_fwd_kernel(const float* __restrict__ x, const float* __restrict__ w,
                                                       float* __restrict__ y, int B, int V, int L, int T,
                                                       int tiles_per_row) {
    __shared__ float wl[CPL * 16];
    int bid = blockIdx.x;
    const int tile = bid % tiles_per_row;
// ... 205 lines not shown
                    const int tp = tpl + r;
                    const bool has_l = (2 * tp - 1) >= 0, has_r = (2 * tp + 1) < Lc;
                    float best = has_l ? fmaxf(c[0][r], 0.f) : -INFINITY;
                    float pre = c[0][r];
                    int sel = 0;
                    const float r1 = fmaxf(c[1][r], 0.f);
                    if (r1 > best) { best = r1; sel = 1; pre = c[1][r]; }
                    if (has_r) {
                        const float r2 = fmaxf(c[2][r], 0.f);
                        if (r2 > best) { best = r2; sel = 2; pre = c[2][r]; }
                    }
                    const float ge = (tp < T && pre > 0.f) ? g4[r] : 0.f;
                    gsel[0][r] = sel == 0 ? ge : 0.f;
                    gsel[1][r] = sel == 1 ? ge : 0.f;
                    gsel[2][r] = sel == 2 ? ge : 0.f;
                }
#pragma unroll
                for (int i = 0; i < 3; ++i)
#pragma unroll
                    for (int r = 0; r < 4; ++r)
                        acc[ct] = __builtin_amdgcn_mfma_f32_16x16x4f32(a2[i + 2 * r], gsel[i][r], acc[ct], 0, 0, 0);
            }
        }
    }
#undef NEF_STEM_GLOAD
#pragma unroll
    for (int ct = 0; ct < 2; ++ct)
#pragma unroll
        for (int r = 0; r < 4; ++r) {
            const int tap = 4 * kk + r;
            if (tap < KW) part[((int64_t)slot * V * CPL + v * CPL + 32 * wave + 16 * ct + n16) * KW + tap] = acc[ct][r];
        }
}

__global__ __launch_bounds__(256) void stem_bwd_weight_reduce(const float* __restrict__ part, float* __restrict__ gw, int n, int nsplit) {
    __shared__ float sm[4][64];
    const int lane = threadIdx.x & 63, wave = threadIdx.x >> 6;
    const int i = blockIdx.x * 64 + lane;
    float s = 0.f;
    if (i < n) {
        for (int sp0 = wave; sp0 < nsplit; sp0 += 32) {
            float v[8];
#pragma unroll
            for (int u = 0; u < 8; ++u) v[u] = sp0 + 4 * u < nsplit ? part[(int64_t)(sp0 + 4 * u) * n + i] : 0.f;
#pragma unroll
            for (int u = 0; u < 8; ++u) s += v[u];
        }
    }
    sm[wave][lane] = s;
    __syncthreads();
    if (wave == 0 && i < n) gw[i] = (sm[0][lane] + sm[1][lane]) + (sm[2][lane] + sm[3][lane]);
}

}

extern "C" {

int nef_stem_fwd(const float* x, const float* w, float* y, int B, int V, int L, nef_stream_t stream) {
    NEF_ENTER();
    NEF_REQUIRE(x && w && y, NEF_E_NULL);
    NEF_REQUIRE(B > 0 && V > 0 && L >= 4 && L % 4 == 0, NEF_E_SHAPE);
    const int T = L / 4;
    const int tiles = (T + FWD_TP - 1) / FWD_TP;
    hipLaunchKernelGGL(stem_fwd_kernel, dim3((unsigned)((int64_t)B * V * tiles)), dim3(256), 0, (hipStream_t)stream, x,
                       w, y, B, V, L, T, tiles);
    return nef_launch_status();
}

size_t nef_stem_bwd_ws_bytes(int V) { return (size_t)(MB_SPLIT > BW_SPLIT ? MB_SPLIT : BW_SPLIT) * V * CPL * KW * sizeof(float); }

int nef_stem_bwd_weight(const float* x, const float* w, const float* gy, float* gw, void* ws, size_t ws_bytes, int B,
                        int V, int L, nef_stream_t stream) {
    NEF_ENTER();
    NEF_REQUIRE(x && w && gy && gw && ws, NEF_E_NULL);
    NEF_REQUIRE(B > 0 && V > 0 && L >= 4 && L % 4 == 0, NEF_E_SHAPE);
    NEF_REQUIRE(ws_bytes >= nef_stem_bwd_ws_bytes(V), NEF_E_WORKSPACE);
    const int T = L / 4;
    hipStream_t st = (hipStream_t)stream;
    const int n = V * CPL * KW;
    const size_t lds = (size_t)(MB_HALO + L + MB_TAIL) * sizeof(float);
    if (T % 2 == 0 && lds <= 64 * 1024) {
        const int slots = B < MB_SPLIT ? B : MB_SPLIT;
        hipLaunchKernelGGL(stem_bwd_weight_mfma_kernel, dim3((unsigned)(slots * V)), dim3(256), lds, st, x, w, gy, (float*)ws, B,
                           V, L, T);
        hipLaunchKernelGGL(stem_bwd_weight_reduce, dim3((n + 63) / 64), dim3(256), 0, st, (const float*)ws, gw, n, slots);
        return nef_launch_status();
    }
    const int tiles = (T + BW_TP - 1) / BW_TP;
    hipLaunchKernelGGL(stem_bwd_weight_kernel, dim3((unsigned)(BW_SPLIT * V * (CPL / BW_CPB))), dim3(256), 0, st, x, w,
                       gy, (float*)ws, B, V, L, T, tiles);
    hipLaunchKernelGGL(stem_bwd_weight_reduce, dim3((n + 63) / 64), dim3(256), 0, st, (const float*)ws, gw, n, BW_SPLIT);
    return nef_launch_status();
}

}
```

electrocardio_panorama_amd/engine.py:

```python
import os

import torch
from . import _env

from . import ops
from .ops import GV

N_SEG, ROI_BINS = 7, 16
DROP_P = 0.2
BN_EPS, BN_MOM = 1e-5, 0.1


DROPOUT_SITES = ("W_encoder.layer1.0", "W_encoder.layer1.1", "W_encoder.layer1.2", "w_conv.0", "z1_conv.0",
                 "z2_conv1.0", "z2_conv2.0", "z2_conv2.2")


class DropCfg:

    def __init__(self, training, p=DROP_P, masks=None, seed=0, seed_dev=None):
        self.seed_dev = seed_dev
        self.on = bool(training) and p > 0.0
        self.p = p if self.on else 0.0
        self.scale = 1.0 / (1.0 - p) if self.on else 1.0
        self.masks = masks
        self.seed = seed

    def windowed(self, site, t0, W):
        if not self.on or self.masks is None:
            return self
        m = dict(self.masks)
        m[site] = self.masks[site][:, :, t0:t0 + W].contiguous()
        return DropCfg(True, self.p, m, self.seed, self.seed_dev)

    def args(self, site):
        if not self.on:
            return dict(mask=None, drop_p=0.0, drop_scale=1.0, seed=0)
        if self.masks is not None:
            return dict(mask=self.masks[site], drop_p=0.0, drop_scale=self.scale, seed=0)
        return dict(mask=None, drop_p=self.p, drop_scale=self.scale, seed_dev=self.seed_dev,
                    seed=(self.seed * 0x9E3779B1 + DROPOUT_SITES.index(site) * 0x85EBCA6B + 1) & 0xFFFFFFFFFFFFFFFF)


def block_fwd(xv, P, prefix, K, Cog, drop, in_scale=None):
    G = xv.G
    h = ops.conv(xv, ops.pack_weight(P[prefix + ".conv1.weight"], G, T=xv.T), Cog, K, relu=True, in_scale=in_scale, **drop.args(prefix))
    res_conv = (K == 3 and Cog != xv.Cg)
    assert in_scale is None or not res_conv
    if res_conv:
        r = ops.conv(xv, ops.pack_weight(P[prefix + ".residual_conv.weight"], G, T=xv.T), Cog, 1,
                     bias=P[prefix + ".residual_conv.bias"])
        resv = GV.dense(r, G)
    else:
        resv = xv
    y = ops.conv(GV.dense(h, G), ops.pack_weight(P[prefix + ".conv2.weight"], G, T=xv.T), Cog, K, res=resv, relu=True,
                 res_scale=in_scale)
    return y, (xv, h, y, prefix, K, Cog, res_conv, drop.scale, in_scale)


def block_scale_ok(P, prefix, G, T):
    return all(ops._pack_shape(P[prefix + n], G, False, T, plain=False)[3] == 3 for n in (".conv1.weight", ".conv2.weight")) and T >= 128


def _bwd_f4(K):
    return K in (3, 7)


def _block_pack_requests(P, prefix, G, T, flip):
    w1 = P[prefix + ".conv1.weight"]
    f4 = bool(flip) and _bwd_f4(w1.shape[2])
    reqs = [ops.PackReq(w1, G, flip, T, f4=f4), ops.PackReq(P[prefix + ".conv2.weight"], G, flip, T, f4=f4)]
    if w1.shape[2] == 3 and w1.shape[0] // G != w1.shape[1]:
        reqs.append(ops.PackReq(P[prefix + ".residual_conv.weight"], G, flip, T))
    return reqs


def _latent_pack_requests(P, V, T, win, flip):
    reqs = []
    for i in range(3):
        reqs += _block_pack_requests(P, f"W_encoder.layer1.{i}", V, T, flip)
    reqs += _block_pack_requests(P, "w_conv.0", V, T, flip)
    reqs += _block_pack_requests(P, "z1_conv.0", V, T, flip)
    reqs += _block_pack_requests(P, "z2_conv1.0", V, win[1] if win is not None else T, flip)
    reqs += _block_pack_requests(P, "z2_conv2.0", N_SEG * V, ROI_BINS, flip)
    reqs += _block_pack_requests(P, "z2_conv2.2", N_SEG * V, 2 * ROI_BINS, flip)
    return reqs


def _decoder_pack_requests(P, T_lat, flip):
    w3 = P["decoder.3.double_conv.0.weight"]
    poly = (ops.poly_bwd_ok if flip else ops.poly_fwd_ok)(1, w3.shape[0], w3.shape[1], 4 * T_lat)
    return ([ops.PackReq(P["decoder.1.double_conv.3.weight"], 1, flip, 2 * T_lat, f4=True)] +
            ([] if poly else [ops.PackReq(w3, 1, flip, 4 * T_lat, f4=True)]) +
            [ops.PackReq(P["decoder.3.double_conv.3.weight"], 1, flip, 4 * T_lat, f4=True)])


def _step_pack_requests(P, V, T):
    r0 = (T - 1) // 2
    win = (r0 - 2, 6) if (T % 2 == 0 and r0 - 2 >= 0 and r0 + 4 <= T) else None
    reqs = _latent_pack_requests(P, V, T, win, False) + _latent_pack_requests(P, V, T, win, True)
    if 2 * T < 128:
        return reqs
    reqs += _decoder_pack_requests(P, T, False) + _decoder_pack_requests(P, T, True)
    w0, w3 = P["decoder.1.double_conv.0.weight"], P["decoder.3.double_conv.0.weight"]
    wg, site0 = _regroup_halves(w0, P), w0.data_ptr()
    co0, co3 = w0.shape[0], w3.shape[0]
    if ops.poly_fwd_ok(2, co0, w0.shape[1] // 2, 2 * T):
        reqs.append(ops.PackReq(wg, 2, False, T, src=("poly", co0), plain=False, site=site0))
    else:
        reqs.append(ops.PackReq(wg, 2, False, 2 * T, f4=True, site=site0))
    if ops.poly_bwd_ok(2, co0, w0.shape[1] // 2, 2 * T):
        reqs.append(ops.PackReq(wg, 2, True, T, src=("poly", 0), site=site0))
    else:
        reqs.append(ops.PackReq(wg, 2, True, 2 * T, f4=True, site=site0))
    if ops.poly_fwd_ok(1, co3, w3.shape[1], 4 * T):
        reqs.append(ops.PackReq(w3, 1, False, 2 * T, src=("poly", co3), plain=False))
    if ops.poly_bwd_ok(1, co3, w3.shape[1], 4 * T):
        reqs.append(ops.PackReq(w3, 1, True, 2 * T, src=("poly", 0)))
    return reqs


_SIDE_MIN_WORK = 1 << 24


def _side(device, work=None):
    mode = _env.get("NEF_SIDE_STREAM", "auto")
    if mode == "0" or (mode == "auto" and work is not None and work < _SIDE_MIN_WORK
                       and not torch.cuda.is_current_stream_capturing()):
        return ops._Inline()
    return ops.SideStream.get(device)


def block_bwd(saved, gy, P, grads, out=None, side=None, pre_gated=False, gate_input=False, scale_bwd=False, g2_chan_sum=None):
    xv, h, y, prefix, K, Cog, res_conv, dscale = saved[:8]
    in_scale = saved[8] if len(saved) > 8 else None
    side = side or ops._Inline()
    G, Cig = xv.G, xv.Cg
    g2 = gy if pre_gated else ops.gate(gy, y)
    g2v, hv = GV.dense(g2, G), GV.dense(h, G)
    grads[prefix + ".conv2.weight"] = side.run(lambda: ops.conv_bwd_weight(hv, g2v, K, site=P[prefix + ".conv2.weight"].data_ptr()), h, g2)
    gc1 = ops.conv(g2v, ops.pack_weight(P[prefix + ".conv2.weight"], G, flip=True, T=xv.T, f4=_bwd_f4(K)), Cog, K, gate=hv,
                   gate_scale=dscale, role="conv_bwd_data")
    gc1v = GV.dense(gc1, G)
    grads[prefix + ".conv1.weight"] = side.run(lambda: ops.conv_bwd_weight(xv, gc1v, K, in_scale=in_scale, site=P[prefix + ".conv1.weight"].data_ptr()), xv.t, gc1)
    if res_conv:
        grads[prefix + ".residual_conv.weight"] = side.run(lambda: ops.conv_bwd_weight(xv, g2v, 1, site=P[prefix + ".residual_conv.weight"].data_ptr()), xv.t, g2)
        grads[prefix + ".residual_conv.bias"] = g2_chan_sum if g2_chan_sum is not None else side.run(lambda: ops.chan_sum(g2), g2)
        gres = ops.conv(g2v, ops.pack_weight(P[prefix + ".residual_conv.weight"], G, flip=True, T=xv.T), Cig, 1,
                        role="conv_bwd_data")
        resv = GV.dense(gres, G)
    else:
        resv = g2v
    wp1f = ops.pack_weight(P[prefix + ".conv1.weight"], G, flip=True, T=xv.T, f4=_bwd_f4(K))
    if in_scale is not None and scale_bwd and int(getattr(wp1f, "nef_wino", 0)) == 3 and out is None:
        slots = ops.conv_stats_buffer(wp1f, xv.B, G, Cig, xv.T, xv.t.device)
        if slots is not None:
            gx = ops.conv(gc1v, wp1f, Cig, K, res=resv, gate=xv, gate_scale=1.0, gate_rowscale=in_scale, stats=slots, stats_mode=1,
                          role="conv_bwd_data")
            return gx, ops.slots_to_rows(slots, xv.B)
    return ops.conv(gc1v, wp1f, Cig, K, res=resv,
                    out=out, gate=xv if gate_input else None, gate_scale=1.0, role="conv_bwd_data")


_DEC = (("decoder.1", "0", "1", 128), ("decoder.1", "3", "4", 128), ("decoder.3", "0", "1", 64),
        ("decoder.3", "3", "4", 64))


_HALVES = "decoder.1.double_conv.0.weight#halves"


def _regroup_halves(w, P=None):
    if P is not None:
        hit = P.get(_HALVES)
        if hit is not None and hit[1] is w and hit[2] == w._version:
            return hit[0]
    wg = ops.regroup_halves(w)
    if P is not None:
        P[_HALVES] = (wg, w, w._version)
    return wg


def _ungroup_halves(w2):
    return ops.regroup_halves(w2, inverse=True)


def _fusable(D, passes):
    return 2 * D.shape[2] >= 128


def _decoder_fwd_unfused(D, P, Bf, passes, training, save):
    x = D
    saved = []
    for li, (blk, cv, bn, cout) in enumerate(_DEC):
        if li in (0, 2):
            x = ops.upsample2_fwd(x)
        wname, bname, pre = f"{blk}.double_conv.{cv}.weight", f"{blk}.double_conv.{cv}.bias", f"{blk}.double_conv.{bn}"
        c = ops.conv(GV.dense(x, 1), ops.pack_weight(P[wname], 1, T=x.shape[2], f4=True), cout, 3, bias=P[bname])
        if training:
            mean, invstd, a, b = ops.bn_train_stats(c, P[pre + ".weight"], P[pre + ".bias"], Bf[pre + ".running_mean"],
                                                    Bf[pre + ".running_var"], passes, BN_EPS, BN_MOM, nbt=Bf[pre + ".num_batches_tracked"])
            np_ = passes
        else:
            a, b = ops.bn_eval_affine(P[pre + ".weight"], P[pre + ".bias"], Bf[pre + ".running_mean"],
                                      Bf[pre + ".running_var"], BN_EPS)
            mean = invstd = None
            np_ = 1
        act = ops.affine_relu_fwd(c, a, b, np_)
        if save:
            saved.append((x, c, mean, invstd, a, b, (0, None, None, 1), li in (0, 2)))
        x = act
    out = ops.outconv_fwd(x, P["decoder.4.weight"], P["decoder.4.bias"])
    return out, (saved, x, out, passes, None)


# ... 108 lines not shown
            gpv, xv = GV.dense(gp2, 2), GV.dense(x, 2)
            if pm:
                grads[wname] = side.run(lambda: _ungroup_halves(ops.conv_bwd_weight_poly(xv, gp2, Cog_, pro, xedge, site=P[wname].data_ptr())), x, gp2, xedge)
            else:
                grads[wname] = side.run(lambda: _ungroup_halves(ops.conv_bwd_weight(xv, gpv, 3, pro=pro, site=P[wname].data_ptr())), x, gp2)
            if poly_b:
                g = ops.conv_bwd_data_poly(gpv, _regroup_halves(P[wname], P), x.shape[1] // 2, site=P[wname].data_ptr(), phase_major=pm)
                poly_first = True
            else:
                g = ops.conv(gpv, ops.pack_weight(_regroup_halves(P[wname], P), 2, flip=True, T=gp2.shape[2], f4=True, site=P[wname].data_ptr()), x.shape[1] // 2, 3,
                             role="conv_bwd_data")
        else:
            gcv, xv = GV.dense(gc, 1), GV.dense(x, 1)
            if pm:
                grads[wname] = side.run(lambda: ops.conv_bwd_weight_poly(xv, gc, Cog_, pro, xedge, site=P[wname].data_ptr()), x, gc, xedge)
            else:
                grads[wname] = side.run(lambda: ops.conv_bwd_weight(xv, gcv, 3, pro=pro, site=P[wname].data_ptr()), x, gc)
            if poly_b:
                bnb = None
                if li > 0 and saved[li - 1][2] is not None:
                    cb, mb, ib, ab, bb = saved[li - 1][1:6]
                    bnb = (cb, mb, ib, ab, bb, cb.shape[0] // passes)
                g = ops.conv_bwd_data_poly(gcv, P[wname], x.shape[1], bnb=bnb, phase_major=pm)
                g_slots = g.nef_slots
                g_is_up = False
                if li == 0:
                    poly_first = True
                continue
            wpf = ops.pack_weight(P[wname], 1, flip=True, T=gc.shape[2], f4=True)
            g_slots = bnb = None
            if li > 0:
                cb, mb, ib, ab, bb = saved[li - 1][1:6]
                Tg = gc.shape[2]
                plain = not up_after and cb.shape[2] == Tg
                upv = bool(up_after) and 2 * cb.shape[2] == Tg and Tg % 8 == 0 and Tg >= 16
                if (plain or upv) and mb is not None:
                    g_slots = ops.conv_stats_buffer(wpf, cb.shape[0], 1, x.shape[1], Tg, gc.device)
                    if g_slots is not None:
                        bnb = (cb, mb, ib, ab, bb, cb.shape[0] // passes, g_slots, upv)
            g = ops.conv(gcv, wpf, x.shape[1], 3, role="conv_bwd_data", bnb=bnb)
        g_is_up = bool(up_after and li > 0 and c.shape[2] % 8 == 0 and c.shape[2] >= 16)
        if up_after and li > 0 and not g_is_up:
            g = ops.upsample2_bwd(g)
    return g, bool(saved[0][7]) and not poly_first, shared_B is not None


def _latents(P, x, in_theta, rois, drop, save, pack_side=None):
    B, V, L = x.shape
    T = L // 4
    sv = {}
    r0 = (T - 1) // 2
    win = (r0 - 2, 6) if (T % 2 == 0 and r0 - 2 >= 0 and r0 + 4 <= T) else None
    ops.pack_many(_latent_pack_requests(P, V, T, win, False))
    a = ops.stem_fwd(x, P["W_encoder.conv1.weight"])
    if pack_side is not None:
        pack_side.join()
    sv["blk_enc"] = []
    for i in range(3):
        a, s = block_fwd(GV.dense(a, V), P, f"W_encoder.layer1.{i}", 7, 128, drop)
        sv["blk_enc"].append(s)
    e = ops.theta_mlp_fwd(in_theta, P["mlp1.weight"], P["mlp1.bias"])
    if block_scale_ok(P, "w_conv.0", V, T):
        enc, sv["blk_w_conv"] = block_fwd(GV.dense(a, V), P, "w_conv.0", 3, 128, drop, in_scale=(e, V * 128, 128))
    else:
        ew = ops.chscale_fwd(a, e)
        enc, sv["blk_w_conv"] = block_fwd(GV.dense(ew, V), P, "w_conv.0", 3, 128, drop)
    z1, sv["blk_z1"] = block_fwd(GV.half(enc, V, 0), P, "z1_conv.0", 3, 128, drop)
    if win is not None:
        xw = ops.window_crop(GV.half(enc, V, 1), win[0], win[1])
        wdrop = drop.windowed("z2_conv1.0", win[0], win[1])
        z2c, sv["blk_z2c"] = block_fwd(GV.dense(xw, V), P, "z2_conv1.0", 3, 128, wdrop)
        z2a = ops.roi_align_fwd(z2c, rois, T, win[0])
    else:
        z2c, sv["blk_z2c"] = block_fwd(GV.half(enc, V, 1), P, "z2_conv1.0", 3, 128, drop)
        z2a = ops.roi_align_fwd(z2c, rois)
    sv["z2_win"] = win
    h0 = z2a.view(B, 128 * V * N_SEG, ROI_BINS)
    h1, sv["blk_c20"] = block_fwd(GV.dense(h0, N_SEG * V), P, "z2_conv2.0", 3, 128, drop)
    h2 = ops.convt2_fwd(h1, P["z2_conv2.1.weight"], P["z2_conv2.1.bias"], N_SEG * V)
    h3, sv["blk_c22"] = block_fwd(GV.dense(h2, N_SEG * V), P, "z2_conv2.2", 3, 128, drop)
    z2b = h3.view(B, 128 * V, N_SEG, 2 * ROI_BINS)
    if save:
        sv.update(x=x, w=a, e=e, in_theta=in_theta, h1=h1, rois=rois, T=T, V=V, B=B)
    return z1, z2b, (sv if save else None)


def _head_shared(T):
    return 2 * T >= 128


def _head_fwd(P, Bf, z1, z2r, q_theta, V, rest_theta, phase, training, lead_choice, sv, rest_chunk, half_sweep, unpool=None):
    B = z1.shape[0]
    save = sv is not None
    q = ops.theta_mlp_fwd(q_theta, P["mlp2.weight"], P["mlp2.bias"])
    z2b = None
    if unpool is not None:
        assert _head_shared(z1.shape[2])
        z2b, rois, status = unpool
        latent, D2 = ops.lead_mean_mix_unpool(z1, z2b, rois, q, V, lead_choice, z1.shape[2], status)
        out3, dsv = decoder_fwd(D2, P, Bf, 3, training, save, shared_B=B)
    elif _head_shared(z1.shape[2]):
        latent, D2 = ops.lead_mean_mix_shared(z1, z2r, q, V, lead_choice)
        out3, dsv = decoder_fwd(D2, P, Bf, 3, training, save, shared_B=B)
    else:
        latent = ops.lead_mean(z1, z2r, V)
        D = ops.mix_fwd(latent, z1, z2r, q, V, lead_choice)
        out3, dsv = decoder_fwd(D, P, Bf, 3, training, save)
    outs = (out3[0:B], out3[B:2 * B], out3[2 * B:3 * B])
    if save:
        sv.update(z1=z1, z2r=z2r, z2b=z2b, latent=latent, q=q, q_theta=q_theta, choice=lead_choice, dec=dsv, hB=B, hV=V)
    if phase == "train":
        return outs, sv
    if phase in ("val", "test"):
        rest = sweep(P, Bf, latent, rest_theta, training, rest_chunk, half_sweep)
        return outs + (rest,), sv
    raise KeyError("please type correct phase")


def _views_fwd(P, Bf, z1, z2r, q_theta, V, training, lead_choice, sv, unpool):
    Q, B, L = q_theta.shape[0], z1.shape[0], 4 * z1.shape[2]
# ... 356 lines not shown
```

electrocardio_panorama_amd/ops.py:

```python
import ctypes as C
import contextlib
import itertools
import os
from typing import NamedTuple, Optional

import torch
from . import _env

from . import _lib

N_SEG, ROI_BINS = 7, 16


def _p(t):
    return None if t is None else t.data_ptr()


def _stream():
    return torch.cuda.current_stream().cuda_stream


def _chk(t, dtype=torch.float32):
    assert t.is_cuda and t.dtype == dtype and t.is_contiguous(), (t.device, t.dtype, t.is_contiguous())
    return t
# ... 73 lines not shown
            self.pending.append((None, inputs))
            return out
        self.pending.append((ev, inputs))
        while self.pending and self.pending[0][0] is not None and self.pending[0][0].query():
            self.pending.pop(0)
        return out

    def join(self):
        torch.cuda.current_stream(self.device).wait_stream(self.stream)
        self.pending.clear()


class _Inline:

    def run(self, fn, *inputs):
        return fn()

    def join(self):
        pass


class GV:
    __slots__ = ("t", "B", "G", "Cg", "T", "bs", "gs", "off")

    def __init__(self, t, B, G, Cg, T, bs, gs, off=0):
        self.t, self.B, self.G, self.Cg, self.T, self.bs, self.gs, self.off = t, B, G, Cg, T, bs, gs, off

    @property
    def ptr(self):
        return self.t.data_ptr() + 4 * self.off

    @staticmethod
    def dense(t, G):
        _chk(t)
        B, Ct, T = t.shape
        return GV(t, B, G, Ct // G, T, Ct * T, (Ct // G) * T, 0)

    @staticmethod
    def half(t, V, which):
        _chk(t)
        B, Ct, T = t.shape
        return GV(t, B, V, 64, T, Ct * T, 128 * T, which * 64 * T)


def stem_fwd(x, w):
    L = _lib.load()
    _chk(x), _chk(w)
    B, V, Ln = x.shape
    y = torch.empty(B, 128 * V, Ln // 4, device=x.device, dtype=torch.float32)
    ev = _hbm("stem_fwd", x, y)
    _lib.check(L.nef_stem_fwd(_p(x), _p(w), _p(y), B, V, Ln, _stream()), "nef_stem_fwd")
    _done(ev)
    return y


def stem_bwd_weight(x, w, gy):
    L = _lib.load()
    _chk(x), _chk(w), _chk(gy)
    B, V, Ln = x.shape
    gw = torch.empty_like(w)
    n = L.nef_stem_bwd_ws_bytes(V)
    ws = workspace(n, x.device)
    ev = _hbm("stem_bwd_weight", x, gy)
    _lib.check(L.nef_stem_bwd_weight(_p(x), _p(w), _p(gy), _p(gw), _p(ws), n, B, V, Ln, _stream()), "nef_stem_bwd_weight")
    _done(ev)
    return gw


_WV = _env.get("NEF_WINOGRAD", "4")
WINOGRAD = _WV != "0"
WINO_FWD = 1 if _WV in ("1", "2") else 2
WINO_BW4 = _WV not in ("1", "2")
WINO_BW7 = _WV not in ("1", "2")


H2 = _env.get("NEF_H2", "1") == "1"


BATCH_HINT = None
_H2_MIN_WGS = 256


def _h2_packed(K, T_out, pro=0):
    return K in (1, 3) and not pro and 8 <= T_out <= 64 and T_out % 4 == 0


def _h2_fills(G, Cout_g, T_out, tile_t, tile_c):
    if BATCH_HINT is None:
        return True
    if T_out < 128:
        spt = (256 + 4) // (T_out + 4)
        return G * ((Cout_g + 63) // 64) * ((BATCH_HINT + spt - 1) // spt) >= _H2_MIN_WGS
    return G * ((Cout_g + tile_c - 1) // tile_c) * BATCH_HINT * ((T_out + tile_t - 1) // tile_t) >= _H2_MIN_WGS


def h2_ok(K, Cin_g, Cout_g, T_out, pro=0):
    return (H2 and (K == 3 or (K in (1, 7) and not pro)) and T_out % 2 == 0 and
            (T_out >= 128 or _h2_packed(K, T_out, pro)) and Cin_g % 16 == 0 and Cout_g % 64 == 0)


H2_FOLLOW_UP = 2.0
H2_FOLLOW_DOWN = 64.0
H2_HEADROOM = 64
H2_TAIL_WINDOW = 2.0 ** -11
H2_TAIL_FRAC = 0.9
H2_TAIL_MODES = ("warn", "fp32")
# ... 325 lines not shown
    _PREPACKED.clear()
    if not reqs:
        return
    for key, r_, wp in zip(keys, reqs, _pack(reqs, "pack_many", align=4)):
        _PREPACKED[key] = (wp, r_[0], r_[0]._version)


def pack_weight(w, G, flip=False, T=None, f4=False, site=None, shared=False, plain=True, src=None):
    _chk(w)
    Cog, Cig, K, wino = _pack_shape(w, G, flip, T, f4, plain, src)
    key = (w.data_ptr(), G, bool(flip), wino, src)
    hit = _PREPACKED.get(key) if _PACK_KEEP else _PREPACKED.pop(key, None)
    if hit is not None and hit[1] is w and hit[2] == w._version:
        return hit[0]
    wp, = _pack([(w, G, Cog, Cig, K, bool(flip), wino, src, site)], "pack_weight")
    if shared:
        wp.nef_shared = True
    return wp


def conv_stats_buffer(wp, B, G, Cog, T_out, device):
    wino = int(getattr(wp, "nef_wino", 0))
    if wino not in (2, 3) or (wino == 3 and T_out < 128):
        return None
    nslot = 2 * ((T_out + 255) // 256) if wino == 3 else _lib.load().nef_conv_stats_slots(T_out, Cog)
    if nslot <= 0:
        return None
    return torch.empty(G * Cog, B * nslot, 2, device=device, dtype=torch.float32), nslot


def bn_stats_from_slots(stats, gamma, beta, running_mean, running_var, P, N, Ln, eps=1e-5, momentum=0.1, nbt=None):
    L = _lib.load()
    slots, nslot = stats
    Ct = slots.shape[0]
    mean, invstd, a, b = (torch.empty(P, Ct, device=slots.device, dtype=torch.float32) for _ in range(4))
    n = L.nef_bn_ws_bytes(P, Ct)
    ws = workspace(n, slots.device)
    _lib.check(L.nef_bn_stats_from_slots(_p(slots), nslot, _p(gamma), _p(beta), _p(running_mean), _p(running_var), _p(mean),
                                         _p(invstd), _p(a), _p(b), _p(ws), n, P, N // P, Ct, Ln, eps, momentum, _p(nbt), _stream()),
               "nef_bn_stats_from_slots")
    return mean, invstd, a, b


def _operand(a, xv, in_scale, pro):
    a.x, a.x_bs, a.x_gs = xv.ptr, xv.bs, xv.gs
    if in_scale is not None:
        a.in_scale, a.sc_bs, a.sc_gs = _p(in_scale[0]), in_scale[1], in_scale[2]
    if pro is not None and pro[0]:
        a.pro_mode, a.pro_a, a.pro_b, a.pro_Bp = pro[0], _p(pro[1]), _p(pro[2]), pro[3]


def conv(xv, wp, Cog, K, out=None, bias=None, in_scale=None, res=None, gate=None, gate_scale=1.0, relu=False,
         mask=None, drop_p=0.0, drop_scale=1.0, seed=0, role="conv_fwd", pro=None, seed_dev=None, stats=None, bnb=None,
         x_scale=0.0, tag_extra="", res_scale=None, gate_rowscale=None, stats_mode=0):
    L = _lib.load()
    T_out = xv.T * 2 if (pro is not None and pro[0] & 2) else xv.T
    if out is None:
        y = torch.empty(xv.B, xv.G * Cog, T_out, device=xv.t.device, dtype=torch.float32)
        out = GV.dense(y, xv.G)
    a = _lib.ConvArgs()
    _operand(a, xv, in_scale, pro)
    a.wp, a.y, a.y_bs, a.y_gs = _p(wp), out.ptr, out.bs, out.gs
    a.bias = _p(bias)
    a.res = res.ptr if res is not None else None
    a.gate = gate.ptr if gate is not None else None
    a.mask = _p(mask)
    if res is not None:
        a.res_bs, a.res_gs = res.bs, res.gs
    if gate_rowscale is not None:
        assert gate is not None
        a.gate_rowscale, a.gr_bs, a.gr_gs = _p(gate_rowscale[0]), gate_rowscale[1], gate_rowscale[2]
    a.stats_mode = int(stats_mode)
    if res_scale is not None:
        assert res is not None
        a.res_scale, a.rs_bs, a.rs_gs = _p(res_scale[0]), res_scale[1], res_scale[2]
    if gate is not None:
        a.gate_bs, a.gate_gs = gate.bs, gate.gs
    a.B, a.T, a.G, a.Cin_g, a.Cout_g, a.K = xv.B, T_out, xv.G, xv.Cg, Cog, K
    a.relu = int(relu)
    a.gate_scale, a.drop_scale, a.drop_p, a.rng_seed = gate_scale, drop_scale, drop_p, seed
    a.rng_seed_dev = _p(seed_dev)
    a.wino = int(getattr(wp, "nef_wino", 0))
    a.x_scale = float(x_scale)
    a.stats = _p(stats[0]) if stats is not None else None
    if bnb is not None:
        a.bnb_x, a.bnb_mean, a.bnb_invstd, a.bnb_a, a.bnb_b = (_p(t) for t in bnb[:5])
        a.bnb_Bp, a.bnb_slots = bnb[5], _p(bnb[6][0])
        a.bnb_up = int(bnb[7]) if len(bnb) > 7 else 0
    if a.wino == 3 and not x_scale:
        st = _amax_state(xv.t.device)
        ws = getattr(wp, "nef_site", None)
        site = None
        if AMAX_SCOPE is not None and ws is not None:
            occ = st["occ"]
            k = occ[(AMAX_SCOPE, ws, role, xv.B, T_out)] = occ.get((AMAX_SCOPE, ws, role, xv.B, T_out), 0) + 1
            site = (AMAX_SCOPE, ws, role, xv.B, T_out, 0 if getattr(wp, "nef_shared", False) else k)
        i = _amax_index(st, site if site is not None else (None, "conv"), 1)
        a.x_amax_next = st["nxt"].data_ptr() + 4 * i
        if i not in st["ready"] or site is None:
            if torch.cuda.is_current_stream_capturing():
                raise RuntimeError("split-fp16 conv: a call site's first launch (it measures its operand) cannot be captured; "
                                   "run the step once eagerly first (GraphedTrainStep does)")
            st["nxt"][i] = 0.0
            _lib.check(L.nef_conv_fwd(C.byref(a), _stream()), "nef_conv_fwd")
            st["cur"][i] = st["nxt"][i]
            if site is not None:
                _note_tail(st, i, [(xv, in_scale, pro)])
            st["ready"].add(i)
        a.x_amax = st["cur"].data_ptr() + 4 * i
        a.x_clamped = st["clamped"].data_ptr()
        st["used"] = True
    extra = ("up" if (pro is not None and pro[0] & 2) else "") + ("ph" if (pro is not None and pro[0] == 4) else "") + ("pf" if (pro is not None and pro[0] & 8) else "") + tag_extra + ("bnb" + ("up" if len(bnb) > 7 and bnb[7] else "") if bnb is not None else "")
    tag = (role, K, xv.G, xv.Cg, Cog, xv.B, T_out) + ((extra,) if extra else ())
    ev = _timed(tag)
    if ev is not None:
        EXEC_FRAC[tag] = 0.0 if a.wino == 3 else _exec_frac(K, a.wino)
        EXEC_FP16[tag] = 3.0 if a.wino == 3 else 0.0
    _lib.check(L.nef_conv_fwd(C.byref(a), _stream()), "nef_conv_fwd")
    if ev is not None:
        ev.record()
    return out.t


def poly_weights(w, tile_Cr=0):
    _chk(w)
    ws = torch.empty(2 * w.shape[0], w.shape[1], 3, device=w.device, dtype=torch.float32)
    _lib.check(_lib.load().nef_poly_weights(_p(w), _p(ws), w.shape[0], w.shape[1], int(tile_Cr), _stream()), "nef_poly_weights")
    return ws


def poly_fwd_ok(G, Cog, Cig, T):
    Th = T // 2
    return (H2 and T % 2 == 0 and Th >= 128 and Cog % 64 == 0 and Cig % 16 == 0 and h2_ok(3, Cig, 2 * Cog, Th, 1) and
            _h2_fills(G, 2 * Cog, Th, 256, 128))


def conv_poly_fwd(xv, w, Cog, bias=None, pro=None, stats=False, site=None, save_edge=False):
    L = _lib.load()
    G, Cig, Th = xv.G, xv.Cg, xv.T
    assert w.shape == (G * Cog, Cig, 3) and xv.bs == G * Cig * Th and xv.gs == Cig * Th, "conv_poly_fwd: dense input rows"
    aff = pro is not None and bool(pro[0] & 1)
    wp = pack_weight(w, G, T=Th, site=w.data_ptr() if site is None else site, plain=False, src=("poly", Cog))
    if int(getattr(wp, "nef_wino", 0)) != 3:
        raise _lib.NefLibraryError("conv_poly_fwd: shape outside the split-fp16 kernel (ask poly_fwd_ok first)")
    y = torch.empty(xv.B, G * Cog, 2 * Th, device=xv.t.device, dtype=torch.float32)
    slots = conv_stats_buffer(wp, xv.B, G, Cog, Th, xv.t.device) if stats else None
    out = GV(y, xv.B, G, 2 * Cog, Th, G * Cog * 2 * Th, Cog * 2 * Th, 0)
    conv(xv, wp, 2 * Cog, 3, out=out, bias=bias, pro=(8 | int(aff), pro[1] if aff else None, pro[2] if aff else None, pro[3] if aff else 1),
         stats=slots)
    pa, pb, pbp = (_p(pro[1]), _p(pro[2]), pro[3]) if aff else (None, None, 1)
    xedge = torch.empty(xv.B, G * Cig, 2, device=xv.t.device, dtype=torch.float32) if save_edge else None
    _lib.check(L.nef_poly_fwd_edge(xv.ptr, _p(w), _p(y), xv.B, G, Cog, Cig, 2 * Th, pa, pb, pbp,
                                   _p(slots[0]) if slots is not None else None, slots[1] if slots is not None else 0, _p(xedge),
                                   _stream()), "nef_poly_fwd_edge")
    y.nef_xedge = xedge
    return (y, slots) if stats else y


def poly_bwd_ok(G, Cog, Cig, T):
    Th = T // 2
    return (H2 and T % 2 == 0 and Th >= 128 and Cig % 64 == 0 and (2 * Cog) % 16 == 0 and h2_ok(3, 2 * Cog, Cig, Th) and
            _h2_fills(G, Cig, Th, 256, 128 if Cig % 128 == 0 else 64))


def conv_bwd_data_poly(gyv, w, Cig, bnb=None, site=None, phase_major=False):
    L = _lib.load()
    if phase_major:
        G, Cog, T = gyv.G, gyv.Cg // 2, 2 * gyv.T
    else:
        G, Cog, T = gyv.G, gyv.Cg, gyv.T
    Th = T // 2
    assert w.shape == (G * Cog, Cig, 3) and gyv.gs == Cog * T, "conv_bwd_data_poly: dense gradient rows"
    wp = pack_weight(w, G, flip=True, T=Th, site=w.data_ptr() if site is None else site, src=("poly", 0))
    if int(getattr(wp, "nef_wino", 0)) != 3:
        raise _lib.NefLibraryError("conv_bwd_data_poly: shape outside the split-fp16 kernel (ask poly_bwd_ok first)")
    xv = GV(gyv.t, gyv.B, G, 2 * Cog, Th, gyv.bs, gyv.gs, gyv.off)
    if bnb is not None and len(bnb) == 6:
        slots = conv_stats_buffer(wp, gyv.B, G, Cig, Th, gyv.t.device)
        bnb = None if slots is None else (*bnb, slots)
    g = conv(xv, wp, Cig, 3, role="conv_bwd_data", bnb=bnb, pro=None if phase_major else (4, None, None, 1),
             tag_extra="pm" if phase_major else "")
    g.nef_slots = bnb[6] if bnb is not None else None
    ba = [None] * 5 + [1, None, 0]
    if bnb is not None:
        ba = [_p(t) for t in bnb[:5]] + [bnb[5], _p(bnb[6][0]), bnb[6][1]]
    _lib.check(L.nef_poly_bwd_edge(gyv.ptr, _p(w), _p(g), gyv.B, G, Cog, Cig, T, *ba, int(phase_major), _stream()), "nef_poly_bwd_edge")
    return g


def poly_w_ok(B, G, Cog, Cig, T):
    Th = T // 2
    return (T % 4 == 0 and Cog % 64 == 0 and h2w_ok(3, Cig, 2 * Cog, Th, 1) and
            (BATCH_HINT is None or B * ((Th + 63) // 64) >= 8 * _H2_MIN_WGS))


def conv_bwd_weight_poly(xv, gy_pm, Cog, pro, xedge, site=None):
    L = _lib.load()
    G, Cig = xv.G, xv.Cg
    aff = pro is not None and bool(pro[0] & 1)
    gyv = GV.dense(gy_pm, G)
    gw2 = conv_bwd_weight(xv, gyv, 3, pro=(4 | int(aff), pro[1] if aff else None, pro[2] if aff else None, pro[3] if aff else 1),
                          site=site, h2=True, xedge=xedge)
    gw = torch.empty(G * Cog, Cig, 3, device=gy_pm.device, dtype=torch.float32)
    n = L.nef_poly_wgrad_fold_ws_bytes(xv.B, G, Cog, Cig)
    ws = torch.empty(n // 4, device=gy_pm.device, dtype=torch.float32)
    _lib.check(L.nef_poly_wgrad_fold(_p(gw2), _p(gy_pm), _p(xedge), _p(gw), _p(ws), n, xv.B, G, Cog, Cig, 2 * xv.T, _stream()),
               "nef_poly_wgrad_fold")
    return gw


def h2w_ok(K, Cig, Cog, T, pro_mode=0, in_scale=False):
    return (H2 and T % 2 == 0 and T >= 64 and Cig % 64 == 0 and Cog % 64 == 0 and
            (K == 3 or not pro_mode) and not (pro_mode and in_scale))


def conv_bwd_weight(xv, gyv, K, in_scale=None, pro=None, wino=None, site=None, h2=None, x_scale=0.0, gy_scale=0.0, xedge=None):
    L = _lib.load()
    B, T, G, Cig, Cog = xv.B, gyv.T, xv.G, xv.Cg, gyv.Cg
    dev = xv.t.device
    gw = torch.empty(G * Cog, Cig, K, device=dev, dtype=torch.float32)
    pm0 = pro[0] if pro is not None else 0
    a = _lib.BwwArgs()
    _operand(a, xv, in_scale, pro)
    a.gy, a.gy_bs, a.gy_gs, a.gw = gyv.ptr, gyv.bs, gyv.gs, _p(gw)
    a.B, a.T, a.G, a.Cin_g, a.Cout_g, a.K = B, T, G, Cig, Cog, K
    a.x_scale, a.gy_scale = float(x_scale), float(gy_scale)
    routed = False
    if h2 is None:
        h2 = (wino is None and h2w_ok(K, Cig, Cog, T, pm0, in_scale is not None) and
              (BATCH_HINT is None or B * ((T + 63) // 64) >= 8 * _H2_MIN_WGS))
    if h2:
        _bww_form(L, a, 3, dev, f"conv_bwd_weight (split-fp16): unsupported shape Cig={Cig} Cog={Cog} K={K} T={T}")
        if not (x_scale and gy_scale):
            st = _amax_state(dev)
            key = None
            if AMAX_SCOPE is not None and site is not None:
                occ = st["occ"]
                base = (AMAX_SCOPE, (site, "w"), "conv_bwd_weight", B, T)
                k = occ[base] = occ.get(base, 0) + 1
                key = base + (k,)
            i = _amax_index(st, key if key is not None else (None, "bww"), 2)
            nxt = st["nxt"].data_ptr() + 4 * i
            a.x_amax_next, a.gy_amax_next = nxt, nxt + 4
            if i not in st["ready"] or key is None:
                if torch.cuda.is_current_stream_capturing():
                    raise RuntimeError("split-fp16 weight gradient: a call site's first launch cannot be captured")
                st["nxt"][i:i + 2] = 0.0
                _bww(L, a)
                st["cur"][i:i + 2] = st["nxt"][i:i + 2]
                if key is not None:
                    flag = _note_tail(st, i, [(xv, in_scale, pro), (gyv, None, None)])
                    if _tail_mode() == "fp32" and int(flag.item()):
                        st["fp32"].add(i)
                        st["fallback"] += 1
                st["ready"].add(i)
            routed = i in st["fp32"]
            if not routed:
                st["used"] = True
                cur = st["cur"].data_ptr() + 4 * i
                a.x_amax, a.gy_amax, a.clamped = cur, cur + 4, st["clamped"].data_ptr()
        if not routed:
            tag = ("conv_bwd_weight", K, G, Cig, Cog, B, T) + (("up",) if pm0 & 2 else (("pw",) if pm0 & 4 else ()))
            ev = _timed(tag)
            if ev is not None:
                EXEC_FRAC[tag] = 0.0
                EXEC_FP16[tag] = 3.0
            _bww(L, a)
            _done(ev)
            return gw
    extra = ("up" if pm0 & 2 else "") + (("pw" if pm0 & 4 else "") + "f32" if routed else "")
    if routed:
        wino = False
    clamp = bool(pm0 & 4)
    if clamp:
        if xedge is None:
            raise _lib.NefLibraryError("conv_bwd_weight: pro_mode bit 2 on the fp32 kernels needs `xedge`")
        pm0 = a.pro_mode = pm0 & 3
    if wino is None:
        wino = (WINOGRAD and ((K == 3 and WINO_BW4) or (K == 7 and WINO_BW7)) and T % 2 == 0 and T >= 64
                and not (K == 7 and pm0))
    wino = 4 if wino else False
    assert wino or not pm0 or in_scale is None
    _bww_form(L, a, wino or 0, dev, f"conv_bwd_weight: unsupported shape Cig={Cig} Cog={Cog} K={K}")
    tag = ("conv_bwd_weight", K, G, Cig, Cog, B, T) + ((extra,) if extra else ())
    ev = _timed(tag)
    if ev is not None:
        EXEC_FRAC[tag] = _exec_frac(K, 2) if wino else 1.0
        EXEC_FP16[tag] = 0.0
    _bww(L, a)
    if clamp:
        assert K == 3 and in_scale is None and tuple(xedge.shape) == (B, G * Cig, 2)
        _lib.check(L.nef_bwd_weight_clamp_ends(_p(xedge), gyv.ptr, gyv.bs, gyv.gs, _p(gw), B, T, G, Cig, Cog, _stream()),
                   "nef_bwd_weight_clamp_ends")
    if ev is not None:
        ev.record()
    return gw


def _bww_form(L, a, form, device, unsupported):
    a.form = form
    a.ws_bytes = L.nef_conv_bwd_weight_ws_bytes(C.byref(a))
    if a.ws_bytes == 0:
        raise _lib.NefLibraryError(unsupported)
    a.ws = _p(workspace(a.ws_bytes, device))


def _bww(L, a):
    _lib.check(L.nef_conv_bwd_weight(C.byref(a), _stream()), "nef_conv_bwd_weight")


def _tail_mode():
    if H2_TAIL_MODE not in H2_TAIL_MODES:
        raise ValueError(f"ops.H2_TAIL_MODE={H2_TAIL_MODE!r}: expected one of {H2_TAIL_MODES}")
    return H2_TAIL_MODE


def chan_sum(x):
    L = _lib.load()
    _chk(x)
    B, Ct, T = x.shape
    out = torch.empty(Ct, device=x.device, dtype=torch.float32)
    n = L.nef_chan_sum_ws_bytes(Ct)
    ws = workspace(n, x.device)
    _lib.check(L.nef_chan_sum(_p(x), _p(out), _p(ws), n, B, Ct, T, _stream()), "nef_chan_sum")
    return out


def _convt2_fma_fwd(x, w, bias, G):
    L = _lib.load()
    _chk(x), _chk(w), _chk(bias)
    B, Ct, T = x.shape
    Cig, Cog = Ct // G, w.shape[1]
    y = torch.empty(B, G * Cog, 2 * T, device=x.device, dtype=torch.float32)
    _lib.check(L.nef_convt2_fwd(_p(x), _p(w), _p(bias), _p(y), B, G, Cig, Cog, T, _stream()), "nef_convt2_fwd")
    return y


def _convt2_fma_bwd_data(gy, w, G):
    L = _lib.load()
    _chk(gy), _chk(w)
    B, Ct, To = gy.shape
    Cog, Cig, T = Ct // G, w.shape[0] // G, To // 2
    gx = torch.empty(B, G * Cig, T, device=gy.device, dtype=torch.float32)
    _lib.check(L.nef_convt2_bwd_data(_p(gy), _p(w), _p(gx), B, G, Cig, Cog, T, _stream()), "nef_convt2_bwd_data")
    return gx


def _convt2_fma_bwd_weight(x, gy, G):
    L = _lib.load()
    _chk(x), _chk(gy)
    B, Ct, T = x.shape
    Cig, Cog = Ct // G, gy.shape[1] // G
    gw = torch.empty(G * Cig, Cog, 2, device=x.device, dtype=torch.float32)
    gb = torch.empty(G * Cog, device=x.device, dtype=torch.float32)
    n = L.nef_convt2_bwd_weight_ws_bytes(G, Cig, Cog)
    ws = workspace(n, x.device)
    _lib.check(L.nef_convt2_bwd_weight(_p(x), _p(gy), _p(gw), _p(gb), _p(ws), n, B, G, Cig, Cog, T, _stream()),
               "nef_convt2_bwd_weight")
    return gw, gb


# ... 1448 lines not shown
```

include/nefnet_hip.h:

```cpp
#ifndef NEFNET_HIP_H
#define NEFNET_HIP_H

#include <stddef.h>
#include <stdint.h>

#ifdef __cplusplus
extern "C" {
#endif

#define NEF_OK 0
#define NEF_E_SHAPE (-1)
#define NEF_E_NULL (-2)
#define NEF_E_WORKSPACE (-3)
#define NEF_E_UNSUPPORTED (-4)

#define NEF_N_SEG 7
#define NEF_ROI_BINS 16

typedef void* nef_stream_t;

int nef_abi_version(void);

int nef_debug_spin_us(float us, int wgs, nef_stream_t stream);

int nef_stem_fwd(const float* x, const float* w, float* y, int B, int V, int L, nef_stream_t stream);
size_t nef_stem_bwd_ws_bytes(int V);
int nef_stem_bwd_weight(const float* x, const float* w, const float* gy, float* gw, void* ws, size_t ws_bytes,
                        int B, int V, int L, nef_stream_t stream);

typedef struct nef_pack_desc {
    const float* w;
    float* wp;
    int32_t G, Cog, Cig, K, transpose_flip, wino;
    int32_t src_mode, src_Cr;
} nef_pack_desc;
size_t nef_pack_bytes(const nef_pack_desc* d);
int nef_pack_weights(const nef_pack_desc* descs, int n, nef_stream_t stream);

typedef struct nef_conv_args {
    const float* x;
    const float* wp;
    float* y;
    const float* bias;
    const float* in_scale;
    const float* res;
    const float* gate;
    const uint8_t* mask;
    int64_t x_bs, x_gs, y_bs, y_gs, sc_bs, sc_gs, res_bs, res_gs, gate_bs, gate_gs;
    int32_t B, T, G, Cin_g, Cout_g, K;
    int32_t relu;
    float gate_scale;
    float drop_scale;
    float drop_p;
    uint64_t rng_seed;
    const float* pro_a;
    const float* pro_b;
    int32_t pro_mode;
    int32_t pro_Bp;
    const uint64_t* rng_seed_dev;
    int32_t wino;
    float* stats;
    const float* bnb_x;
    const float* bnb_mean;
    const float* bnb_invstd;
    const float* bnb_a;
    const float* bnb_b;
    float* bnb_slots;
    int32_t bnb_Bp;
    int32_t bnb_up;
    float x_scale;
    int32_t reserved0;
    const float* x_amax;
    float* x_amax_next;
    int32_t* x_clamped;
    const float* res_scale;
    int64_t rs_bs, rs_gs;
    const float* gate_rowscale;
    int64_t gr_bs, gr_gs;
    int32_t stats_mode;
    int32_t reserved1;
} nef_conv_args;

int nef_conv_fwd(const nef_conv_args* a, nef_stream_t stream);
size_t nef_conv_args_bytes(void);

typedef struct nef_bww_args {
    const float* x;
    const float* gy;
    float* gw;
    void* ws;
    const float* in_scale;
    const float* pro_a;
    const float* pro_b;
    const float* x_amax;
    const float* gy_amax;
    float* x_amax_next;
    float* gy_amax_next;
    int32_t* clamped;
    size_t ws_bytes;
    int64_t x_bs, x_gs, gy_bs, gy_gs, sc_bs, sc_gs;
    int32_t B, T, G, Cin_g, Cout_g, K;
    int32_t pro_mode;
    int32_t pro_Bp;
    int32_t form;
    float x_scale;
    float gy_scale;
    int32_t reserved0;
} nef_bww_args;

int nef_conv_bwd_weight(const nef_bww_args* a, nef_stream_t stream);
size_t nef_conv_bwd_weight_ws_bytes(const nef_bww_args* a);
size_t nef_bww_args_bytes(void);

typedef struct nef_h2_tail_census_out {
    uint64_t n_nonzero, n_small;
    double e_small, e_total;
    float frac_count, frac_energy;
    int32_t flag, reserved;
} nef_h2_tail_census_out;
size_t nef_h2_tail_census_ws_bytes(int B, int G, int Cg);
int nef_h2_tail_census(const float* x, int64_t x_bs, int64_t x_gs, int B, int G, int Cg, int T, const float* in_scale, int64_t sc_bs,
                       int64_t sc_gs, const float* pro_a, const float* pro_b, int pro_mode, int pro_Bp, const float* amax, float window,
                       float frac, void* ws, size_t ws_bytes, nef_h2_tail_census_out* out, int32_t* site_flag, float* tail_stat,
                       nef_stream_t stream);
int nef_bwd_weight_clamp_ends(const float* xedge, const float* gy, int64_t gy_bs, int64_t gy_gs, float* gw, int B, int T, int G,
                              int Cin_g, int Cout_g, nef_stream_t stream);

size_t nef_chan_sum_ws_bytes(int C);
int nef_chan_sum(const float* x, float* out, void* ws, size_t ws_bytes, int B, int C, int T, nef_stream_t stream);

int nef_convt2_fwd(const float* x, const float* w, const float* bias, float* y, int B, int G, int Cig, int Cog,
                   int T, nef_stream_t stream);
int nef_convt2_bwd_data(const float* gy, const float* w, float* gx, int B, int G, int Cig, int Cog, int T,
                        nef_stream_t stream);
int nef_group_transpose(const float* in, float* out, int G, int R, int Cn, nef_stream_t stream);
int nef_convt2_interleave(const float* yq, const float* bias, float* y, int B, int C, int T, nef_stream_t stream);
int nef_convt2_deinterleave(const float* gy, float* gyq, int B, int C, int T, nef_stream_t stream);
size_t nef_convt2_bwd_weight_ws_bytes(int G, int Cig, int Cog);
int nef_convt2_bwd_weight(const float* x, const float* gy, float* gw, float* gb, void* ws, size_t ws_bytes, int B,
                          int G, int Cig, int Cog, int T, nef_stream_t stream);

int nef_theta_mlp_fwd(const float* theta, const float* W, const float* bias, float* y, int N, int O,
                      nef_stream_t stream);
int nef_theta_mlp_bwd(const float* theta, const float* gy, float* gW, float* gb, int N, int O, nef_stream_t stream);
int nef_theta_encode(const float* theta, float* enc, int N, nef_stream_t stream);

int nef_chscale_fwd(const float* x, const float* s, int64_t s_bs, float* y, int B, int C, int T, nef_stream_t stream);
int nef_chscale_bwd(const float* gy, const float* x, const float* s, int64_t s_bs, float* gx, float* gs, int B,
                    int C, int T, int relu_x, nef_stream_t stream);

int nef_gate(const float* g, const float* ref, float* out, float scale, int64_t n, nef_stream_t stream);
int nef_add(const float* a, const float* b, float* out, int64_t n, nef_stream_t stream);
int nef_window_crop(const float* src, int64_t x_bs, int64_t x_gs, float* dst, int B, int G, int Cg, int T, int t0, int W,
                    nef_stream_t stream);
int nef_window_scatter(const float* src, float* dst, int64_t y_bs, int64_t y_gs, int B, int G, int Cg, int T, int t0,
                       int W, nef_stream_t stream);

int nef_roi_align_fwd(const float* z, const int64_t* rois, float* out, int B, int C, int T, int zT, int t_off,
                      nef_stream_t stream);
int nef_roi_align_bwd(const float* gout, const int64_t* rois, float* gz, int B, int C, int T, int zT, int t_off,
                      nef_stream_t stream);
int nef_roi_unpool_fwd(const float* zseg, const int64_t* rois, float* out, int32_t* status, int B, int C, int T,
                       nef_stream_t stream);
// ... 490 lines not shown
```

Before: 9073.

## Skip conv tiles in beats' all-zero tails using per-item live extents

A new kernel computes, for each batch item and lead, how far its signal is nonzero. The encoder-side split-fp16 forward and backward-data convs then zero their buffer extents and skip the MFMA loop for tiles that lie entirely past that extent. The weight-gradient kernel gets compacted per-group tile lists, built by a prefix-sum kernel, so its teams iterate only over live tiles. This removes arithmetic on padded zero regions at the cost of extra small kernels, extra workspace and a data-dependent amount of work, which depends on the input really having zero tails.

```diff
diff --git a/electrocardio_panorama_amd/_env.py b/electrocardio_panorama_amd/_env.py
--- a/electrocardio_panorama_amd/_env.py
+++ b/electrocardio_panorama_amd/_env.py
@@ -6,6 +6,8 @@
     "NEF_H2_TAIL": "warn (default): split-fp16 call sites whose operand is heavy-tailed (ops.H2_TAIL_FRAC) are counted and reported; "
                    "fp32: such WEIGHT-GRADIENT sites run on the fp32 kernels for their lifetime (per site, per rank)",
     "NEF_H2_ALLOW_CLAMP": "1: Solver warns instead of raising when a split-fp16 launch clamped outside a protected train step",
+    "NEF_LIVE": "1 (default): the encoder-side convs skip the tiles in a beat's all-zero tail (ops.LIVE / ops.LIVE_WGRAD); fwd: forward and "
+                "backward-data convs only, the weight gradients multiply every item; 0: off",
     "NEF_WINOGRAD": "fp32 path: 4 (default) F(4,.) forms where allowed, 2 / 1: F(2,.) only, 0: direct kernels only",
     "NEF_SIDE_STREAM": "auto (default) / 1 / 0: weight gradients on a second HIP stream",
     "NEF_SOLVER_GRAPH": "0: Solver never replays the captured step",
diff --git a/electrocardio_panorama_amd/_lib.py b/electrocardio_panorama_amd/_lib.py
--- a/electrocardio_panorama_amd/_lib.py
+++ b/electrocardio_panorama_amd/_lib.py
@@ -156,10 +156,13 @@
     "nef_stem_bwd_weight": (i32, [p, p, p, p, p, sz, i32, i32, i32, p]),
     "nef_pack_weights": (i32, [C.POINTER(PackDesc), i32, p]),
     "nef_pack_bytes": (sz, [C.POINTER(PackDesc)]),
+    "nef_live_extent": (i32, [p, p, i32, i32, i32, p]),
     "nef_conv_fwd": (i32, [C.POINTER(ConvArgs), p]),
+    "nef_conv_fwd_live": (i32, [C.POINTER(ConvArgs), p, i32, p]),
     "nef_conv_args_bytes": (sz, []),
     "nef_conv_bwd_weight_ws_bytes": (sz, [C.POINTER(BwwArgs)]),
     "nef_conv_bwd_weight": (i32, [C.POINTER(BwwArgs), p]),
+    "nef_conv_bwd_weight_live": (i32, [C.POINTER(BwwArgs), p, i32, p]),
     "nef_bww_args_bytes": (sz, []),
     "nef_h2_tail_census_ws_bytes": (sz, [i32, i32, i32]),
     "nef_h2_tail_census": (i32, [p, i64, i64, i32, i32, i32, i32, p, i64, i64, p, p, i32, i32, p, f32, f32, p, sz, p, p, p, p]),
diff --git a/electrocardio_panorama_amd/csrc/conv_h2.hip b/electrocardio_panorama_amd/csrc/conv_h2.hip
--- a/electrocardio_panorama_amd/csrc/conv_h2.hip
+++ b/electrocardio_panorama_amd/csrc/conv_h2.hip
@@ -114,7 +114,8 @@
 #define NEF_H2_TRACK2(V, W) amax_ = fmaxf(amax_, fmaxf(fabsf(V), fabsf(W)));
 constexpr int H2_OCC1 = 3;
 template <int K, int PRO, int TM, bool PACK = false>
-__global__ __launch_bounds__(256, (TM == 1 && (PRO & 2) == 0) ? H2_OCC1 : 2) void conv_h2_kernel(nef_conv_args a_, int tps_, int n_tiles_, int m_tiles_) {
+__global__ __launch_bounds__(256, (TM == 1 && (PRO & 2) == 0) ? H2_OCC1 : 2) void conv_h2_kernel(nef_conv_args a_, int tps_, int n_tiles_, int m_tiles_,
+                                                                                                const int32_t* live_, int live_add_) {
     constexpr int MT = 64 * TM;
     constexpr bool UP = (PRO & 2) != 0, AFF = (PRO & 1) != 0;
     constexpr bool PH = (PRO & 4) != 0;
@@ -139,7 +140,7 @@
 
     typedef const nef_conv_args __attribute__((address_space(4))) kargs_t;
     auto tile_pass = [&](kargs_t* const ap, const int bid, const int tid, const int tps, const int n_tiles, const int m_tiles,
-                         const float xs_force, const bool last) __attribute__((always_inline)) -> float {
+                         const float xs_force, const bool last, const int32_t* const lv, const int lv_add) __attribute__((always_inline)) -> float {
 #define a (*ap)
     const int tile = bid % n_tiles;
     const int gm = bid / n_tiles;
@@ -162,6 +163,11 @@
     }
     const int m0 = mt * MT;
     const int T = a.T, Cig = a.Cin_g, Cog = a.Cout_g;
+    bool dead = false;
+    if constexpr (PRO == 0 && !PACK) {
+        if (lv) dead = t0 - PAD >= lv[b0 * a.G + g] + lv_add;
+    }
+    const unsigned op_bytes = dead ? 0u : 0x7FFFFFFCu;
     const int lane = tid & 63, wave = tid >> 6;
     const int lo = lane & 31, hi = lane >> 5;
     const int wave_u = __builtin_amdgcn_readfirstlane(wave);
@@ -169,10 +175,10 @@
     const int Tin = UP ? (T >> 1) : (PH ? 2 * T : T);
 
     const float* const xbase = a.x + (int64_t)b0 * a.x_bs + (int64_t)g * a.x_gs;
-    const __amdgpu_buffer_rsrc_t xrs = nef_rsrc(xbase);
+    const __amdgpu_buffer_rsrc_t xrs = nef_rsrc_n(xbase, op_bytes);
     const _Float16* const wph = reinterpret_cast<const _Float16*>(a.wp);
     const int ncot = Cog / 32, nc16 = Cig / 16;
-    const __amdgpu_buffer_rsrc_t wrs = nef_rsrc(wph + ((int64_t)g * nc16 * K * ncot * 2 + (int64_t)(m0 / 32 + TM * wm) * 2) * 512);
+    const __amdgpu_buffer_rsrc_t wrs = nef_rsrc_n(wph + ((int64_t)g * nc16 * K * ncot * 2 + (int64_t)(m0 / 32 + TM * wm) * 2) * 512, op_bytes);
     const unsigned a_tap = (unsigned)(ncot * 2 * 1024);
 
     const int64_t soff = (int64_t)b0 * a.sc_bs + (int64_t)g * a.sc_gs;
@@ -395,7 +401,7 @@
     NEF_H2X_STORE(0, Xl)
     __syncthreads();
 
-    const int nst = Cig / KC;
+    const int nst = dead ? 0 : Cig / KC;
     const unsigned fb_lane = (unsigned)(hi * HALF + (wn * 32 + lo) * 16);
     for (int st = 0; st < nst; ++st) {
         const unsigned char* const xb = Xl + (st & 1) * (2 * PLANE) + fb_lane;
@@ -454,7 +460,7 @@
         __syncthreads();
     }
     {
-        const float wg_ = fmaxf(fmaxf(Al[0], Al[1]), fmaxf(Al[2], Al[3]));
+        const float wg_ = dead ? 0.f : fmaxf(fmaxf(Al[0], Al[1]), fmaxf(Al[2], Al[3]));
         if (!last && !(wg_ * xs_ < 65000.f) && wg_ < 3e38f) {
             __syncthreads();
             return wg_;
@@ -753,19 +759,19 @@
     };
     kargs_t* ap_ = (kargs_t*)__builtin_amdgcn_kernarg_segment_ptr();
     (void)a_;
-    const float over_ = tile_pass(ap_, (int)blockIdx.x, (int)threadIdx.x, tps_, n_tiles_, m_tiles_, 0.f, false);
+    const float over_ = tile_pass(ap_, (int)blockIdx.x, (int)threadIdx.x, tps_, n_tiles_, m_tiles_, 0.f, false, live_, live_add_);
     if (over_ > 0.f) {
         int e_;
         (void)frexpf(over_, &e_);
         int bid_ = (int)blockIdx.x, tid_ = (int)threadIdx.x, tps2_ = tps_, nt2_ = n_tiles_, mt2_ = m_tiles_;
         asm volatile("" : "+s"(ap_), "+s"(bid_), "+s"(tps2_), "+s"(nt2_), "+s"(mt2_));
         asm volatile("" : "+v"(tid_));
-        (void)tile_pass(ap_, bid_, tid_, tps2_, nt2_, mt2_, ldexpf(1.f, 9 - e_ < 100 ? 9 - e_ : 100), true);
+        (void)tile_pass(ap_, bid_, tid_, tps2_, nt2_, mt2_, ldexpf(1.f, 9 - e_ < 100 ? 9 - e_ : 100), true, nullptr, 0);
     }
 }
 
 template <int K, int PRO, int TM, bool PACK = false>
-int launch_h2(const nef_conv_args& a, hipStream_t st) {
+int launch_h2(const nef_conv_args& a, hipStream_t st, const int32_t* live = nullptr, int live_add = 0) {
     constexpr int MT = 64 * TM;
     constexpr int XROW = NTO + K - 1;
     constexpr int P4 = (XROW + 3) / 4 + 1;
@@ -778,7 +784,7 @@
     const int m_tiles = a.Cout_g / MT;
     const int64_t blocks = (int64_t)a.G * m_tiles * n_tiles;
     if (blocks <= 0 || blocks > 0x7fffffff) return NEF_E_SHAPE;
-    hipLaunchKernelGGL((conv_h2_kernel<K, PRO, TM, PACK>), dim3((unsigned)blocks), dim3(256), lds, st, a, tps, n_tiles, m_tiles);
+    hipLaunchKernelGGL((conv_h2_kernel<K, PRO, TM, PACK>), dim3((unsigned)blocks), dim3(256), lds, st, a, tps, n_tiles, m_tiles, live, live_add);
     return nef_launch_status();
 }
 
@@ -805,16 +811,16 @@
            (!(a->pro_mode & 1) || a->Cin_g <= PRO_MAX_CIN);
 }
 
-__attribute__((visibility("hidden"))) int nef_h2_launch(const nef_conv_args* a, hipStream_t st) {
+__attribute__((visibility("hidden"))) int nef_h2_launch(const nef_conv_args* a, hipStream_t st, const int32_t* live, int live_add) {
     if (!nef_h2_ok(a)) return NEF_E_SHAPE;
     if ((a->pro_mode & 1) && !(a->pro_a && a->pro_b && a->pro_Bp > 0)) return NEF_E_NULL;
     const bool wide = a->Cout_g % 128 == 0;
     if (a->T < NTO / 2)
         return a->K == 1 ? launch_h2<1, 0, 1, true>(*a, st) : launch_h2<3, 0, 1, true>(*a, st);
-    if (a->K == 7) return wide ? launch_h2<7, 0, 2>(*a, st) : launch_h2<7, 0, 1>(*a, st);
-    if (a->K == 1) return wide ? launch_h2<1, 0, 2>(*a, st) : launch_h2<1, 0, 1>(*a, st);
+    if (a->K == 7) return wide ? launch_h2<7, 0, 2>(*a, st, live, live_add) : launch_h2<7, 0, 1>(*a, st, live, live_add);
+    if (a->K == 1) return wide ? launch_h2<1, 0, 2>(*a, st, live, live_add) : launch_h2<1, 0, 1>(*a, st, live, live_add);
     switch (a->pro_mode) {
-        case 0: return wide ? launch_h2<3, 0, 2>(*a, st) : launch_h2<3, 0, 1>(*a, st);
+        case 0: return wide ? launch_h2<3, 0, 2>(*a, st, live, live_add) : launch_h2<3, 0, 1>(*a, st, live, live_add);
         case 1: return wide ? launch_h2<3, 1, 2>(*a, st) : launch_h2<3, 1, 1>(*a, st);
         case 2: return launch_h2<3, 2, 1>(*a, st);
         case 4: return wide ? launch_h2<3, 4, 2>(*a, st) : launch_h2<3, 4, 1>(*a, st);
diff --git a/electrocardio_panorama_amd/csrc/conv_h2w.hip b/electrocardio_panorama_amd/csrc/conv_h2w.hip
--- a/electrocardio_panorama_amd/csrc/conv_h2w.hip
+++ b/electrocardio_panorama_amd/csrc/conv_h2w.hip
@@ -42,7 +42,50 @@
     int B, T, G, Cig, Cog, pro_Bp, S, tps, n_tiles, m_tiles, c_tiles, teams;
     float x_scale, gy_scale;
     int xclamp;
+    const int32_t* live_rank;
+    const int32_t* live_items;
 };
+
+__global__ __launch_bounds__(256) void h2w_live_tables_kernel(const int32_t* __restrict__ live, int add, int B, int G, int tps,
+                                                              int32_t* __restrict__ rank, int32_t* __restrict__ items) {
+    extern __shared__ int pre_[];
+    __shared__ int sc_[256];
+    const int g = blockIdx.x;
+    const int n_tiles = B * tps;
+    const int tid = (int)threadIdx.x;
+    int carry = 0;
+    for (int base = 0; base < B; base += 256) {
+        const int b = base + tid;
+        int c = 0;
+        if (b < B) {
+            const int bound = live[b * G + g] + add;
+            c = bound > 0 ? (bound + TT - 1) / TT : 0;
+            c = c < tps ? c : tps;
+        }
+        sc_[tid] = c;
+        __syncthreads();
+        for (int o = 1; o < 256; o <<= 1) {
+            const int v = tid >= o ? sc_[tid - o] : 0;
+            __syncthreads();
+            sc_[tid] += v;
+            __syncthreads();
+        }
+        if (b < B) pre_[b + 1] = carry + sc_[tid];
+        carry += sc_[255];
+        __syncthreads();
+    }
+    if (tid == 0) pre_[0] = 0;
+    __syncthreads();
+    int32_t* const rk = rank + (int64_t)g * (n_tiles + 1);
+    int32_t* const it = items + (int64_t)g * n_tiles;
+    for (int N = threadIdx.x; N < n_tiles; N += 256) {
+        const int b = N / tps, tile = N - b * tps;
+        const int p0 = pre_[b], c = pre_[b + 1] - p0;
+        rk[N] = p0 + (tile < c ? tile : c);
+        if (tile < c) it[p0 + tile] = N;
+    }
+    if (threadIdx.x == 0) rk[n_tiles] = pre_[B];
+}
 
 
 __device__ __forceinline__ void split_pair_s(float x0, float x1, float s, unsigned& h, unsigned& l) {
@@ -452,6 +495,23 @@
     const int n_lo = (int)(per * sp);
     int n_hi = (int)(per * (sp + 1));
     if (n_hi > a.n_tiles) n_hi = a.n_tiles;
+    const int32_t* items_ = nullptr;
+    int ioff_ = 0;
+    if constexpr (PRO == 0) {
+        if (a.live_rank && n_lo < n_hi) {
+            const int32_t* const rk = a.live_rank + (int64_t)g * (a.n_tiles + 1);
+            const int j_lo = rk[n_lo], j_hi = rk[n_hi];
+            items_ = a.live_items + (int64_t)g * a.n_tiles;
+            ioff_ = j_lo - n_lo;
+            n_hi = n_lo + (j_hi - j_lo);
+        }
+    }
+    auto item = [&](int N) __attribute__((always_inline)) -> int {
+        if constexpr (PRO == 0) {
+            if (items_) return N < n_hi ? items_[N + ioff_] : 0;
+        }
+        return N;
+    };
 
     float* const Wl = reinterpret_cast<float*>(smem_w);
     float rx_ = 0.f, rg_ = 0.f;
@@ -487,11 +547,12 @@
     };
     Stage st0, st1;
 
-    auto is_edge = [&](int N) { const int t0_ = (N % a.tps) * TTv; return !(t0_ > 0 && t0_ + TTv + 6 <= T); };
+    auto is_edge = [&](int N) { const int t0_ = (item(N) % a.tps) * TTv; return !(t0_ > 0 && t0_ + TTv + 6 <= T); };
 
     auto issue = [&](Stage& z, int N, auto edge_c, int part) __attribute__((always_inline)) {
         constexpr bool EDGE = decltype(edge_c)::value;
-        const int b_ = N / a.tps, t0_ = (N % a.tps) * TTv;
+        const int Ni_ = item(N);
+        const int b_ = Ni_ / a.tps, t0_ = (Ni_ % a.tps) * TTv;
         const bool on_ = N < n_hi;
         const int64_t goff = (int64_t)b_ * a.gy_bs + (int64_t)g * a.gy_gs + (int64_t)(mt * RG) * T + (EDGE ? 0 : t0_);
         const __amdgpu_buffer_rsrc_t grs = nef_rsrc_n(a.gy + goff, extent_from(a.gy_end, goff, on_));
@@ -549,7 +610,7 @@
 
     auto store = [&](Stage& z, int N, unsigned char* bufp, auto edge_c, int part) __attribute__((always_inline)) {
         constexpr bool EDGE = decltype(edge_c)::value;
-        const int t0_ = (N % a.tps) * TTv;
+        const int t0_ = (item(N) % a.tps) * TTv;
 #pragma unroll
         for (int q = 0; q < ((part & 1) ? NGQ : 0); ++q) {
             const f32x4 v = z.gq[q];
@@ -756,7 +817,13 @@
     return S;
 }
 
-__attribute__((visibility("hidden"))) int nef_h2w_launch(const nef_bww_args& b, int S, hipStream_t st) {
+__attribute__((visibility("hidden"))) size_t nef_h2w_live_bytes(int B, int T, int G) {
+    const int64_t n_tiles = (int64_t)B * ((T + TT - 1) / TT);
+    return (size_t)G * (2 * n_tiles + 1) * sizeof(int32_t);
+}
+
+__attribute__((visibility("hidden"))) int nef_h2w_launch(const nef_bww_args& b, int S, hipStream_t st, const int32_t* live, int live_add,
+                                                          void* tables) {
     const int B = b.B, T = b.T, G = b.G, Cig = b.Cin_g, Cog = b.Cout_g, K = b.K;
     int pro_mode = b.pro_mode;
     if (!nef_h2w_ok(B, T, Cig, Cog, K, pro_mode)) return NEF_E_SHAPE;
@@ -773,6 +840,14 @@
     a.teams = G * S;
     a.x_scale = b.x_scale, a.gy_scale = b.gy_scale;
     a.xclamp = (pro_mode >> 2) & 1;
+    a.live_rank = a.live_items = nullptr;
+    if (live && tables && pro_mode == 0 && h2w2_form(Cog, 0) && (size_t)(B + 1) * sizeof(int) <= 48 * 1024) {
+        int32_t* const rank = static_cast<int32_t*>(tables);
+        int32_t* const items = rank + (int64_t)G * ((int64_t)a.n_tiles + 1);
+        hipLaunchKernelGGL(h2w_live_tables_kernel, dim3((unsigned)G), dim3(256), (size_t)(B + 1) * sizeof(int), st, live, live_add, B, G,
+                           a.tps, rank, items);
+        a.live_rank = rank, a.live_items = items;
+    }
     pro_mode &= 3;
     const int Tin = (pro_mode & 2) ? T / 2 : T;
     a.x_end = ((int64_t)(B - 1) * b.x_bs + (int64_t)(G - 1) * b.x_gs + (int64_t)Cig * Tin) * 4;
diff --git a/electrocardio_panorama_amd/csrc/conv_mfma.hip b/electrocardio_panorama_amd/csrc/conv_mfma.hip
--- a/electrocardio_panorama_amd/csrc/conv_mfma.hip
+++ b/electrocardio_panorama_amd/csrc/conv_mfma.hip
@@ -1958,7 +1958,7 @@
 }
 
 __attribute__((visibility("hidden"))) bool nef_h2_ok(const nef_conv_args* a);
-__attribute__((visibility("hidden"))) int nef_h2_launch(const nef_conv_args* a, hipStream_t st);
+__attribute__((visibility("hidden"))) int nef_h2_launch(const nef_conv_args* a, hipStream_t st, const int32_t* live, int live_add);
 __attribute__((visibility("hidden"))) int nef_h2_pack(const nef_pack_desc* descs, int n, hipStream_t st);
 __attribute__((visibility("hidden"))) int nef_h2_pack_status(const nef_pack_desc* d);
 
@@ -2032,8 +2032,7 @@
 size_t nef_conv_args_bytes(void) { return sizeof(nef_conv_args); }
 
 
-int nef_conv_fwd(const nef_conv_args* a, nef_stream_t stream) {
-    NEF_ENTER();
+static int conv_fwd_entry(const nef_conv_args* a, const int32_t* live, int32_t live_add, nef_stream_t stream) {
     NEF_REQUIRE(a && a->x && a->wp && a->y, NEF_E_NULL);
     NEF_REQUIRE(a->B > 0 && a->T > 0 && a->G > 0, NEF_E_SHAPE);
     const int K = a->K;
@@ -2048,7 +2047,7 @@
     NEF_REQUIRE((!a->res_scale && !a->gate_rowscale && a->stats_mode == 0) || a->wino == 3, NEF_E_UNSUPPORTED);
     if (a->wino == 3) {
         NEF_REQUIRE(nef_h2_ok(a), NEF_E_SHAPE);
-        return nef_h2_launch(a, st);
+        return nef_h2_launch(a, st, live, live_add);
     }
     bool big = (a->Cout_g % 128 == 0);
     if (big) {
@@ -2079,6 +2078,17 @@
         case 3: return big ? launch_conv_fwd<3, 2>(*a, st) : launch_conv_fwd<3, 1>(*a, st);
         default: return big ? launch_conv_fwd<1, 2>(*a, st) : launch_conv_fwd<1, 1>(*a, st);
     }
+}
+
+int nef_conv_fwd(const nef_conv_args* a, nef_stream_t stream) {
+    NEF_ENTER();
+    return conv_fwd_entry(a, nullptr, 0, stream);
+}
+
+int nef_conv_fwd_live(const nef_conv_args* a, const int32_t* live, int32_t live_add, nef_stream_t stream) {
+    NEF_ENTER();
+    NEF_REQUIRE(live, NEF_E_NULL);
+    return conv_fwd_entry(a, live, live_add, stream);
 }
 
 int nef_conv_stats_slots(int T, int Cout_g) {
@@ -2107,7 +2117,7 @@
             if (p_ > partials) partials = p_;
         }
     }
-    return (size_t)partials * G * K * Cout_g * Cin_g * sizeof(float);
+    return (size_t)partials * G * K * Cout_g * Cin_g * sizeof(float) + (a->form == 3 && partials ? nef_h2w_live_bytes(B, T, G) : 0);
 }
 
 static int bww_direct(const nef_bww_args& a, hipStream_t st, int* S_used) {
@@ -2145,16 +2155,16 @@
     return rc;
 }
 
-static int bww_h2(const nef_bww_args& a, hipStream_t st, int* S_used) {
+static int bww_h2(const nef_bww_args& a, hipStream_t st, int* S_used, const int32_t* live, int live_add) {
     NEF_REQUIRE(a.G > 0 && nef_h2w_ok(a.B, a.T, a.Cin_g, a.Cout_g, a.K, a.pro_mode), NEF_E_SHAPE);
     NEF_REQUIRE(!(a.pro_mode && a.in_scale), NEF_E_UNSUPPORTED);
     const int S = nef_h2w_splits(a.B, a.T, a.G, a.Cin_g, a.Cout_g, a.K, a.pro_mode, S_used);
-    NEF_REQUIRE(a.ws_bytes >= (size_t)*S_used * a.G * a.K * a.Cout_g * a.Cin_g * sizeof(float), NEF_E_WORKSPACE);
-    return nef_h2w_launch(a, S, st);
-}
-
-int nef_conv_bwd_weight(const nef_bww_args* args, nef_stream_t stream) {
-    NEF_ENTER();
+    const size_t partial_bytes = (size_t)*S_used * a.G * a.K * a.Cout_g * a.Cin_g * sizeof(float);
+    NEF_REQUIRE(a.ws_bytes >= partial_bytes + (live ? nef_h2w_live_bytes(a.B, a.T, a.G) : 0), NEF_E_WORKSPACE);
+    return nef_h2w_launch(a, S, st, live, live_add, live ? static_cast<char*>(a.ws) + partial_bytes : nullptr);
+}
+
+static int conv_bwd_weight_entry(const nef_bww_args* args, const int32_t* live, int32_t live_add, nef_stream_t stream) {
     NEF_REQUIRE(args && args->x && args->gy && args->gw && args->ws, NEF_E_NULL);
     nef_bww_args a = *args;
     if (!(a.pro_mode & 1) && a.pro_Bp <= 0) a.pro_Bp = 1;
@@ -2164,7 +2174,7 @@
     switch (a.form) {
         case 0: rc = bww_direct(a, st, &S); break;
         case 4: rc = nef_mfma_bww_wino4(a, st, &S); break;
-        case 3: rc = bww_h2(a, st, &S); break;
+        case 3: rc = bww_h2(a, st, &S, live, live_add); break;
         default: return NEF_E_UNSUPPORTED;
     }
     if (rc != NEF_OK) return rc;
@@ -2172,6 +2182,18 @@
     hipLaunchKernelGGL(conv_bwd_weight_reduce, dim3(nef_stream_grid(n, 256)), dim3(256), 0, st, (const float*)a.ws, a.gw, a.G,
                        a.Cout_g, a.Cin_g, a.K, S);
     return nef_launch_status();
+}
+
+int nef_conv_bwd_weight(const nef_bww_args* args, nef_stream_t stream) {
+    NEF_ENTER();
+    return conv_bwd_weight_entry(args, nullptr, 0, stream);
+}
+
+int nef_conv_bwd_weight_live(const nef_bww_args* args, const int32_t* live, int32_t live_add, nef_stream_t stream) {
+    NEF_ENTER();
+    NEF_REQUIRE(args && live, NEF_E_NULL);
+    NEF_REQUIRE(args->form == 3, NEF_E_UNSUPPORTED);
+    return conv_bwd_weight_entry(args, live, live_add, stream);
 }
 
 size_t nef_chan_sum_ws_bytes(int C) { return (size_t)CHAN_SUM_SPLIT * C * sizeof(double); }
diff --git a/electrocardio_panorama_amd/csrc/nef_common.h b/electrocardio_panorama_amd/csrc/nef_common.h
--- a/electrocardio_panorama_amd/csrc/nef_common.h
+++ b/electrocardio_panorama_amd/csrc/nef_common.h
@@ -121,7 +121,8 @@
 extern "C" {
 NEF_HIDDEN bool nef_h2w_ok(int B, int T, int Cig, int Cog, int K, int pro_mode);
 NEF_HIDDEN int nef_h2w_splits(int B, int T, int G, int Cig, int Cog, int K, int pro_mode, int* partials);
-NEF_HIDDEN int nef_h2w_launch(const nef_bww_args& a, int S, hipStream_t st);
+NEF_HIDDEN int nef_h2w_launch(const nef_bww_args& a, int S, hipStream_t st, const int32_t* live, int live_add, void* tables);
+NEF_HIDDEN size_t nef_h2w_live_bytes(int B, int T, int G);
 NEF_HIDDEN bool nef_bww_glds_ok(const nef_bww_args& a);
 NEF_HIDDEN int nef_bww_glds_launch(const nef_bww_args& a, int half, int S_max, int fixed_S, int* S_used, hipStream_t st);
 }
diff --git a/electrocardio_panorama_amd/csrc/stem.hip b/electrocardio_panorama_amd/csrc/stem.hip
--- a/electrocardio_panorama_amd/csrc/stem.hip
+++ b/electrocardio_panorama_amd/csrc/stem.hip
@@ -281,9 +281,54 @@
     if (wave == 0 && i < n) gw[i] = (sm[0][lane] + sm[1][lane]) + (sm[2][lane] + sm[3][lane]);
 }
 
+__global__ __launch_bounds__(256) void live_extent_kernel(const float* __restrict__ x, int32_t* __restrict__ live, int L, int vec) {
+    __shared__ int sm[4];
+    const float* const row = x + (int64_t)blockIdx.x * L;
+    int e = 0;
+    if (vec) {
+        const float4* const row4 = reinterpret_cast<const float4*>(row);
+        for (int i = threadIdx.x; i < L / 4; i += 256) {
+            const float4 v = row4[i];
+            const int m = v.w != 0.f ? 4 : (v.z != 0.f ? 3 : (v.y != 0.f ? 2 : (v.x != 0.f ? 1 : 0)));
+            if (m) e = 4 * i + m;
+        }
+    } else {
+        for (int i = threadIdx.x; i < L; i += 256)
+            if (row[i] != 0.f) e = i + 1;
+    }
+#pragma unroll
+    for (int o = 32; o > 0; o >>= 1) {
+        const int t = __shfl_xor(e, o, 64);
+        e = t > e ? t : e;
+    }
+    if ((threadIdx.x & 63) == 0) sm[threadIdx.x >> 6] = e;
+    __syncthreads();
+    if (threadIdx.x == 0) {
+        const int a = sm[0] > sm[1] ? sm[0] : sm[1], b = sm[2] > sm[3] ? sm[2] : sm[3];
+        e = a > b ? a : b;
+        int cj = 0, lv = 0;
+        if (e) {
+            cj = (e + 6) / 2 + 1;
+            cj = cj < L / 2 ? cj : L / 2;
+            lv = cj / 2 + 1;
+            lv = lv < L / 4 ? lv : L / 4;
+        }
+        live[blockIdx.x] = lv;
+    }
+}
+
 }
 
 extern "C" {
+
+int nef_live_extent(const float* x, int32_t* live, int B, int V, int L, nef_stream_t stream) {
+    NEF_ENTER();
+    NEF_REQUIRE(x && live, NEF_E_NULL);
+    NEF_REQUIRE(B > 0 && V > 0 && L >= 4 && L % 4 == 0 && (int64_t)B * V <= 0x7fffffff, NEF_E_SHAPE);
+    const int vec = (reinterpret_cast<uintptr_t>(x) & 15) == 0;
+    hipLaunchKernelGGL(live_extent_kernel, dim3((unsigned)(B * V)), dim3(256), 0, (hipStream_t)stream, x, live, L, vec);
+    return nef_launch_status();
+}
 
 int nef_stem_fwd(const float* x, const float* w, float* y, int B, int V, int L, nef_stream_t stream) {
     NEF_ENTER();
diff --git a/electrocardio_panorama_amd/engine.py b/electrocardio_panorama_amd/engine.py
--- a/electrocardio_panorama_amd/engine.py
+++ b/electrocardio_panorama_amd/engine.py
@@ -41,20 +41,30 @@
                     seed=(self.seed * 0x9E3779B1 + DROPOUT_SITES.index(site) * 0x85EBCA6B + 1) & 0xFFFFFFFFFFFFFFFF)
 
 
-def block_fwd(xv, P, prefix, K, Cog, drop, in_scale=None):
+def _live_add(live, n):
+    return None if live is None else (live[0], live[1] + n)
+
+
+def block_live_out(saved):
+    live = saved[9] if len(saved) > 9 else None
+    return None if saved[6] else _live_add(live, 2 * ((saved[4] - 1) // 2))
+
+
+def block_fwd(xv, P, prefix, K, Cog, drop, in_scale=None, live=None):
     G = xv.G
-    h = ops.conv(xv, ops.pack_weight(P[prefix + ".conv1.weight"], G, T=xv.T), Cog, K, relu=True, in_scale=in_scale, **drop.args(prefix))
+    h = ops.conv(xv, ops.pack_weight(P[prefix + ".conv1.weight"], G, T=xv.T), Cog, K, relu=True, in_scale=in_scale, live=live,
+                 **drop.args(prefix))
     res_conv = (K == 3 and Cog != xv.Cg)
     assert in_scale is None or not res_conv
     if res_conv:
         r = ops.conv(xv, ops.pack_weight(P[prefix + ".residual_conv.weight"], G, T=xv.T), Cog, 1,
-                     bias=P[prefix + ".residual_conv.bias"])
+                     bias=P[prefix + ".residual_conv.bias"], live=live)
         resv = GV.dense(r, G)
     else:
         resv = xv
     y = ops.conv(GV.dense(h, G), ops.pack_weight(P[prefix + ".conv2.weight"], G, T=xv.T), Cog, K, res=resv, relu=True,
-                 res_scale=in_scale)
-    return y, (xv, h, y, prefix, K, Cog, res_conv, drop.scale, in_scale)
+                 res_scale=in_scale, live=_live_add(live, (K - 1) // 2))
+    return y, (xv, h, y, prefix, K, Cog, res_conv, drop.scale, in_scale, live)
 
 
 def block_scale_ok(P, prefix, G, T):
@@ -133,15 +143,18 @@
 def block_bwd(saved, gy, P, grads, out=None, side=None, pre_gated=False, gate_input=False, scale_bwd=False, g2_chan_sum=None):
     xv, h, y, prefix, K, Cog, res_conv, dscale = saved[:8]
     in_scale = saved[8] if len(saved) > 8 else None
+    live_x = saved[9] if len(saved) > 9 else None
+    live_h = _live_add(live_x, (K - 1) // 2)
+    live_y = block_live_out(saved)
     side = side or ops._Inline()
     G, Cig = xv.G, xv.Cg
     g2 = gy if pre_gated else ops.gate(gy, y)
     g2v, hv = GV.dense(g2, G), GV.dense(h, G)
-    grads[prefix + ".conv2.weight"] = side.run(lambda: ops.conv_bwd_weight(hv, g2v, K, site=P[prefix + ".conv2.weight"].data_ptr()), h, g2)
+    grads[prefix + ".conv2.weight"] = side.run(lambda: ops.conv_bwd_weight(hv, g2v, K, site=P[prefix + ".conv2.weight"].data_ptr(), live=live_y), h, g2)
     gc1 = ops.conv(g2v, ops.pack_weight(P[prefix + ".conv2.weight"], G, flip=True, T=xv.T, f4=_bwd_f4(K)), Cog, K, gate=hv,
-                   gate_scale=dscale, role="conv_bwd_data")
+                   gate_scale=dscale, role="conv_bwd_data", live=live_y)
     gc1v = GV.dense(gc1, G)
-    grads[prefix + ".conv1.weight"] = side.run(lambda: ops.conv_bwd_weight(xv, gc1v, K, in_scale=in_scale, site=P[prefix + ".conv1.weight"].data_ptr()), xv.t, gc1)
+    grads[prefix + ".conv1.weight"] = side.run(lambda: ops.conv_bwd_weight(xv, gc1v, K, in_scale=in_scale, site=P[prefix + ".conv1.weight"].data_ptr(), live=live_h), xv.t, gc1)
     if res_conv:
         grads[prefix + ".residual_conv.weight"] = side.run(lambda: ops.conv_bwd_weight(xv, g2v, 1, site=P[prefix + ".residual_conv.weight"].data_ptr()), xv.t, g2)
         grads[prefix + ".residual_conv.bias"] = g2_chan_sum if g2_chan_sum is not None else side.run(lambda: ops.chan_sum(g2), g2)
@@ -155,10 +168,10 @@
         slots = ops.conv_stats_buffer(wp1f, xv.B, G, Cig, xv.T, xv.t.device)
         if slots is not None:
             gx = ops.conv(gc1v, wp1f, Cig, K, res=resv, gate=xv, gate_scale=1.0, gate_rowscale=in_scale, stats=slots, stats_mode=1,
-                          role="conv_bwd_data")
+                          role="conv_bwd_data", live=live_h)
             return gx, ops.slots_to_rows(slots, xv.B)
     return ops.conv(gc1v, wp1f, Cig, K, res=resv,
-                    out=out, gate=xv if gate_input else None, gate_scale=1.0, role="conv_bwd_data")
+                    out=out, gate=xv if gate_input else None, gate_scale=1.0, role="conv_bwd_data", live=live_h)
 
 
 _DEC = (("decoder.1", "0", "1", 128), ("decoder.1", "3", "4", 128), ("decoder.3", "0", "1", 64),
@@ -373,20 +386,23 @@
     r0 = (T - 1) // 2
     win = (r0 - 2, 6) if (T % 2 == 0 and r0 - 2 >= 0 and r0 + 4 <= T) else None
     ops.pack_many(_latent_pack_requests(P, V, T, win, False))
+    live = (ops.live_extent(x), 0) if ops.LIVE else None
     a = ops.stem_fwd(x, P["W_encoder.conv1.weight"])
     if pack_side is not None:
         pack_side.join()
     sv["blk_enc"] = []
     for i in range(3):
-        a, s = block_fwd(GV.dense(a, V), P, f"W_encoder.layer1.{i}", 7, 128, drop)
+        a, s = block_fwd(GV.dense(a, V), P, f"W_encoder.layer1.{i}", 7, 128, drop, live=live)
         sv["blk_enc"].append(s)
+        live = block_live_out(s)
     e = ops.theta_mlp_fwd(in_theta, P["mlp1.weight"], P["mlp1.bias"])
     if block_scale_ok(P, "w_conv.0", V, T):
-        enc, sv["blk_w_conv"] = block_fwd(GV.dense(a, V), P, "w_conv.0", 3, 128, drop, in_scale=(e, V * 128, 128))
+        enc, sv["blk_w_conv"] = block_fwd(GV.dense(a, V), P, "w_conv.0", 3, 128, drop, in_scale=(e, V * 128, 128), live=live)
     else:
         ew = ops.chscale_fwd(a, e)
-        enc, sv["blk_w_conv"] = block_fwd(GV.dense(ew, V), P, "w_conv.0", 3, 128, drop)
-    z1, sv["blk_z1"] = block_fwd(GV.half(enc, V, 0), P, "z1_conv.0", 3, 128, drop)
+        enc, sv["blk_w_conv"] = block_fwd(GV.dense(ew, V), P, "w_conv.0", 3, 128, drop, live=live)
+    live = block_live_out(sv["blk_w_conv"])
+    z1, sv["blk_z1"] = block_fwd(GV.half(enc, V, 0), P, "z1_conv.0", 3, 128, drop, live=live)
     if win is not None:
         xw = ops.window_crop(GV.half(enc, V, 1), win[0], win[1])
         wdrop = drop.windowed("z2_conv1.0", win[0], win[1])
diff --git a/electrocardio_panorama_amd/ops.py b/electrocardio_panorama_amd/ops.py
--- a/electrocardio_panorama_amd/ops.py
+++ b/electrocardio_panorama_amd/ops.py
@@ -149,6 +149,45 @@
     _lib.check(L.nef_stem_fwd(_p(x), _p(w), _p(y), B, V, Ln, _stream()), "nef_stem_fwd")
     _done(ev)
     return y
+
+
+_LV = _env.get("NEF_LIVE", "1")
+if _LV not in ("0", "1", "fwd"):
+    raise ValueError(f"NEF_LIVE={_LV!r}: expected 0, 1 or fwd")
+LIVE = _LV != "0"
+LIVE_WGRAD = _LV == "1"
+_LIVE_HOST = [None, None]
+_LIVE_ACC = {}
+_LIVE_ACC_OF = [None]
+
+
+def live_extent(x):
+    L = _lib.load()
+    _chk(x)
+    B, V, Ln = x.shape
+    live = torch.empty(B, V, device=x.device, dtype=torch.int32)
+    ev = _hbm("live_extent", x)
+    _lib.check(L.nef_live_extent(_p(x), _p(live), B, V, Ln, _stream()), "nef_live_extent")
+    _done(ev)
+    return live
+
+
+def _live_note(tag, frac):
+    if _LIVE_ACC_OF[0] is not PROFILE:
+        _LIVE_ACC.clear()
+        _LIVE_ACC_OF[0] = PROFILE
+    acc = _LIVE_ACC.setdefault(tag, [0.0, 0])
+    acc[0] += frac
+    acc[1] += 1
+    EXEC_FP16[tag] = 3.0 * acc[0] / acc[1]
+
+
+def _live_frac(live, pad, T, tile=256):
+    if _LIVE_HOST[0] is not live[0]:
+        _LIVE_HOST[0], _LIVE_HOST[1] = live[0], live[0].to("cpu", torch.int64)
+    tps = (T + tile - 1) // tile
+    bound = _LIVE_HOST[1] + int(live[1]) + pad
+    return float(((bound + tile - 1) // tile).clamp(0, tps).double().mean()) / tps
 
 
 def stem_bwd_weight(x, w, gy):
@@ -580,8 +619,16 @@
 
 def conv(xv, wp, Cog, K, out=None, bias=None, in_scale=None, res=None, gate=None, gate_scale=1.0, relu=False,
          mask=None, drop_p=0.0, drop_scale=1.0, seed=0, role="conv_fwd", pro=None, seed_dev=None, stats=None, bnb=None,
-         x_scale=0.0, tag_extra="", res_scale=None, gate_rowscale=None, stats_mode=0):
-    L = _lib.load()
+         x_scale=0.0, tag_extra="", res_scale=None, gate_rowscale=None, stats_mode=0, live=None):
+    L = _lib.load()
+    if live is not None and not LIVE:
+        live = None
+
+    def launch():
+        if live is not None:
+            _lib.check(L.nef_conv_fwd_live(C.byref(a), _p(live[0]), int(live[1]), _stream()), "nef_conv_fwd_live")
+        else:
+            _lib.check(L.nef_conv_fwd(C.byref(a), _stream()), "nef_conv_fwd")
     T_out = xv.T * 2 if (pro is not None and pro[0] & 2) else xv.T
     if out is None:
         y = torch.empty(xv.B, xv.G * Cog, T_out, device=xv.t.device, dtype=torch.float32)
@@ -630,7 +677,7 @@
                 raise RuntimeError("split-fp16 conv: a call site's first launch (it measures its operand) cannot be captured; "
                                    "run the step once eagerly first (GraphedTrainStep does)")
             st["nxt"][i] = 0.0
-            _lib.check(L.nef_conv_fwd(C.byref(a), _stream()), "nef_conv_fwd")
+            launch()
             st["cur"][i] = st["nxt"][i]
             if site is not None:
                 _note_tail(st, i, [(xv, in_scale, pro)])
@@ -640,11 +687,16 @@
         st["used"] = True
     extra = ("up" if (pro is not None and pro[0] & 2) else "") + ("ph" if (pro is not None and pro[0] == 4) else "") + ("pf" if (pro is not None and pro[0] & 8) else "") + tag_extra + ("bnb" + ("up" if len(bnb) > 7 and bnb[7] else "") if bnb is not None else "")
     tag = (role, K, xv.G, xv.Cg, Cog, xv.B, T_out) + ((extra,) if extra else ())
+    frac = 1.0
+    if PROFILE is not None and live is not None and a.wino == 3 and not a.pro_mode and T_out >= 128:
+        frac = _live_frac(live, (K - 1) // 2, T_out)
     ev = _timed(tag)
     if ev is not None:
         EXEC_FRAC[tag] = 0.0 if a.wino == 3 else _exec_frac(K, a.wino)
         EXEC_FP16[tag] = 3.0 if a.wino == 3 else 0.0
-    _lib.check(L.nef_conv_fwd(C.byref(a), _stream()), "nef_conv_fwd")
+        if a.wino == 3 and LIVE:
+            _live_note(tag, frac)
+    launch()
     if ev is not None:
         ev.record()
     return out.t
@@ -742,7 +794,7 @@
             (K == 3 or not pro_mode) and not (pro_mode and in_scale))
 
 
-def conv_bwd_weight(xv, gyv, K, in_scale=None, pro=None, wino=None, site=None, h2=None, x_scale=0.0, gy_scale=0.0, xedge=None):
+def conv_bwd_weight(xv, gyv, K, in_scale=None, pro=None, wino=None, site=None, h2=None, x_scale=0.0, gy_scale=0.0, xedge=None, live=None):
     L = _lib.load()
     B, T, G, Cig, Cog = xv.B, gyv.T, xv.G, xv.Cg, gyv.Cg
     dev = xv.t.device
@@ -774,7 +826,7 @@
                 if torch.cuda.is_current_stream_capturing():
                     raise RuntimeError("split-fp16 weight gradient: a call site's first launch cannot be captured")
                 st["nxt"][i:i + 2] = 0.0
-                _bww(L, a)
+                _bww(L, a, live)
                 st["cur"][i:i + 2] = st["nxt"][i:i + 2]
                 if key is not None:
                     flag = _note_tail(st, i, [(xv, in_scale, pro), (gyv, None, None)])
@@ -789,11 +841,16 @@
                 a.x_amax, a.gy_amax, a.clamped = cur, cur + 4, st["clamped"].data_ptr()
         if not routed:
             tag = ("conv_bwd_weight", K, G, Cig, Cog, B, T) + (("up",) if pm0 & 2 else (("pw",) if pm0 & 4 else ()))
+            frac = 1.0
+            if PROFILE is not None and live is not None and LIVE and LIVE_WGRAD and not pm0 and Cog % 128 == 0:
+                frac = _live_frac(live, 0, T, 64)
             ev = _timed(tag)
             if ev is not None:
                 EXEC_FRAC[tag] = 0.0
                 EXEC_FP16[tag] = 3.0
-            _bww(L, a)
+                if LIVE:
+                    _live_note(tag, frac)
+            _bww(L, a, live)
             _done(ev)
             return gw
     extra = ("up" if pm0 & 2 else "") + (("pw" if pm0 & 4 else "") + "f32" if routed else "")
@@ -833,8 +890,11 @@
     a.ws = _p(workspace(a.ws_bytes, device))
 
 
-def _bww(L, a):
-    _lib.check(L.nef_conv_bwd_weight(C.byref(a), _stream()), "nef_conv_bwd_weight")
+def _bww(L, a, live=None):
+    if live is not None and LIVE and LIVE_WGRAD and a.form == 3:
+        _lib.check(L.nef_conv_bwd_weight_live(C.byref(a), _p(live[0]), int(live[1]), _stream()), "nef_conv_bwd_weight_live")
+    else:
+        _lib.check(L.nef_conv_bwd_weight(C.byref(a), _stream()), "nef_conv_bwd_weight")
 
 
 def _tail_mode():
diff --git a/include/nefnet_hip.h b/include/nefnet_hip.h
--- a/include/nefnet_hip.h
+++ b/include/nefnet_hip.h
@@ -24,6 +24,7 @@
 int nef_debug_spin_us(float us, int wgs, nef_stream_t stream);
 
 int nef_stem_fwd(const float* x, const float* w, float* y, int B, int V, int L, nef_stream_t stream);
+int nef_live_extent(const float* x, int32_t* live, int B, int V, int L, nef_stream_t stream);
 size_t nef_stem_bwd_ws_bytes(int V);
 int nef_stem_bwd_weight(const float* x, const float* w, const float* gy, float* gw, void* ws, size_t ws_bytes,
                         int B, int V, int L, nef_stream_t stream);
@@ -82,6 +83,7 @@
 } nef_conv_args;
 
 int nef_conv_fwd(const nef_conv_args* a, nef_stream_t stream);
+int nef_conv_fwd_live(const nef_conv_args* a, const int32_t* live, int32_t live_add, nef_stream_t stream);
 size_t nef_conv_args_bytes(void);
 
 typedef struct nef_bww_args {
@@ -109,6 +111,7 @@
 } nef_bww_args;
 
 int nef_conv_bwd_weight(const nef_bww_args* a, nef_stream_t stream);
+int nef_conv_bwd_weight_live(const nef_bww_args* a, const int32_t* live, int32_t live_add, nef_stream_t stream);
 size_t nef_conv_bwd_weight_ws_bytes(const nef_bww_args* a);
 size_t nef_bww_args_bytes(void);
 
```

Result: faster. 9973, median of 6 (+9.9%).
